# shanice-l/UNOPose

Measured on AMD Instinct MI355X. Metric: (query,ref) pairs/sec forward, higher is better.
Workload: dtype bf16; 1 GPU; UNOPose.forward, batch 32 pairs/GPU, 2048 query pts, 5000->2048 reference pts, 196 coarse pts, 518x518 crops, DINOv2 ViT-B/14 reg4, random-init (trained-like) weights

## Files before the change

### include/unopose_hip.h

```cpp
#ifndef UNOPOSE_HIP_H
#define UNOPOSE_HIP_H

#include <stdint.h>

#ifdef __cplusplus
extern "C" {
#endif

#define UNOPOSE_OK 0
#define UNOPOSE_EINVAL 1
#define UNOPOSE_ELAUNCH 2
#define UNOPOSE_ENOMEM 3

typedef void *unopose_stream_t;

int unopose_abi_version(void);
const char *unopose_last_error(void);


int unopose_furthest_point_sampling(const float *xyz, int B, int N, int M,
                                    int32_t *idx, unopose_stream_t stream);

int unopose_gather_points(const float *points, const int32_t *idx, int B, int C,
                          int N, int M, float *out, unopose_stream_t stream);

int unopose_gather_points_grad(const float *grad_out, const int32_t *idx, int B,
                               int C, int N, int M, float *grad_points,
                               unopose_stream_t stream);

int unopose_ball_query(const float *new_xyz, const float *xyz, int B, int N,
                       int M, float radius, int nsample, int32_t *idx,
                       unopose_stream_t stream);

int unopose_group_points(const float *points, const int32_t *idx, int B, int C,
                         int N, int M, int S, float *out,
                         unopose_stream_t stream);

int unopose_group_points_grad(const float *grad_out, const int32_t *idx, int B,
                              int C, int N, int M, int S, float *grad_points,
                              unopose_stream_t stream);

int unopose_three_nn(const float *unknown, const float *known, int B, int n,
                     int m, float *dist2, int32_t *idx, unopose_stream_t stream);

int unopose_three_interpolate(const float *points, const int32_t *idx,
                              const float *weight, int B, int c, int m, int n,
                              float *out, unopose_stream_t stream);

int unopose_three_interpolate_grad(const float *grad_out, const int32_t *idx,
                                   const float *weight, int B, int c, int n,
                                   int m, float *grad_points,
                                   unopose_stream_t stream);


int unopose_lrf_global(const float *pts, int B, int N, int use_ref_rad,
                       float *out, unopose_stream_t stream);

int unopose_query_lrf_group(const float *xyz, int B, int N, float radius,
                            int nsample, float *out, unopose_stream_t stream);

int unopose_lrf_group_idx(const float *xyz, const float *new_xyz, const int *idx,
                          int B, int N, float radius, int nsample, float *out,
                          unopose_stream_t stream);

int unopose_weighted_procrustes(const float *src, const float *ref,
                                const float *w, int M, int N, float thresh,
                                float eps, float *R, float *t,
                                unopose_stream_t stream);

int unopose_pe_image_bytes(void);
int unopose_pe_pack_weights(const float *w1, const float *b1, const float *w2, const float *b2,
                            const float *w3, const float *b3, void *image, unopose_stream_t stream);
int unopose_pe_group_mlp_max_packed(const float *xyz, int B, int N, float radius, int nsample,
                                    const void *image, float *out, unopose_stream_t stream);

int unopose_pe_group_mlp_max_packed_cand(const float *xyz, int B, int N, float radius, int nsample,
                                         const void *image, const int *cand_in, const int *cand_cnt_in,
                                         int cand_stride, int *cand_out, int *cand_cnt_out, float *out,
                                         unopose_stream_t stream);
int unopose_pe_group_mlp_max_packed_out(const float *xyz, int B, int N, float radius, int nsample, const void *image,
                                        const int *cand_in, const int *cand_cnt_in, int cand_stride, int *cand_out,
                                        int *cand_cnt_out, void *out, int out_ld, int out_split, unopose_stream_t stream);

int unopose_geo_embedding(const float *points, int B, int n, const void *wd_hi,
                          const void *wd_lo, const void *wa_hi, const void *wa_lo,
                          const float *bias_sum, const float *div_term,
                          float sigma_d, float factor_a, int reduce_mean, int split,
                          int out_bf16, int32_t *knn_ws, void *out,
                          unopose_stream_t stream);

int unopose_geo_embedding_table(const float *points, int B, int n, const float *tab_d, int rows_d, const float *tab_a, int rows_a,
                                const float *bias_sum, const float *w_d, const float *div_term, int hinv, int npoint, float sigma_d,
                                float factor_a, int reduce_mean, int out_bf16, int32_t *knn_ws, void *out,
                                unopose_stream_t stream);

int unopose_geo_embedding_train_workgroups(int B, int n);
int unopose_geo_embedding_train_forward(const float *points, int B, int n, const float *tab_d, int rows_d, const float *tab_a, int rows_a,
                                        const float *bias_sum, const float *w_d, const float *div_term, int hinv, float sigma_d, float factor_a,
                                        int reduce_mean, int32_t *knn, float *out, void *amax, unopose_stream_t stream);
int unopose_geo_embedding_train_backward(const float *points, const int32_t *knn, int B, int n, int rows_d, int rows_a, int hinv, float sigma_d,
                                         float factor_a, int reduce_mean, const float *dE, const void *amax, float *ws, float *full_d,
                                         int *past_table, unopose_stream_t stream);

int unopose_pe_group_mlp_max(const float *xyz, int B, int N, float radius, int nsample,
                             const float *w1, const float *b1, const float *w2,
                             const float *b2, const float *w3, const float *b3,
                             int bf16x3, float *out, unopose_stream_t stream);

int unopose_softmax_stats(const float *x, int B, int R, int C, float *stats_ws, unopose_stream_t stream);
int unopose_infonce_grad(const float *x, int B, int R, int C, const float *stats_ws, const long long *label1,
                         const long long *label2, const float *g, float *grad, unopose_stream_t stream);

int unopose_bn_train_chunk(void);
int unopose_bn_relu_train_forward(const float *x, int B, int C, long L, const float *gamma, const float *beta, float eps, float momentum,
                                  float *running_mean, float *running_var, float *workspace, float *mean, float *rstd, float *y,
                                  unopose_stream_t stream);
int unopose_bn_relu_train_backward(const float *x, const float *dy, int B, int C, long L, const float *gamma, const float *beta,
                                   const float *mean, const float *rstd, float *workspace, float *dgamma, float *dbeta, float *dx,
                                   unopose_stream_t stream);

int unopose_bn_relu_maxpool_train_forward(const float *x, int B, int C, int N, int S, const float *gamma, const float *beta, float eps,
                                          float momentum, float *running_mean, float *running_var, float *workspace, float *mean, float *rstd,
                                          float *out, int32_t *idx, unopose_stream_t stream);
int unopose_bn_relu_maxpool_train_backward(const float *x, const float *g, const int32_t *idx, int B, int C, int N, int S, const float *gamma,
                                           const float *beta, const float *mean, const float *rstd, float *workspace, float *dgamma, float *dbeta,
                                           float *dx, unopose_stream_t stream);

int unopose_saliency_train_forward(const float *atten, const float *s1, const float *s2, int B, int n1, int n2, float *m1, float *m2, float *rmax,
                                   float *rsum, float *cmax, float *csum, unopose_stream_t stream);
int unopose_saliency_train_backward(const float *atten, const float *s1, const float *s2, const float *m1, const float *m2, const float *rmax,
                                    const float *rsum, const float *cmax, const float *csum, const float *g1, const float *g2, int B, int n1, int n2,
                                    float *d_atten, float *ds1, float *ds2, unopose_stream_t stream);

int unopose_nearest_partner(const float *a, const float *b, int B, int n, int m, int over_b, float thr, float *dmin, int32_t *arg,
                            uint8_t *any_close, unopose_stream_t stream);

int unopose_conv1x1_train_wgrad_blocks(void);
int unopose_conv1x1_train_forward(const float *x, int B, int cin, long L, const float *w, int cout, float *y, unopose_stream_t stream);
int unopose_conv1x1_train_wgrad(const float *dy, const float *x, int B, int cout, int cin, long L, float *workspace, float *dw,
                                unopose_stream_t stream);

int unopose_linear_wgrad_f32_splits(long rows, int N, int K);
int unopose_linear_wgrad_f32(const float *g, const float *x, long rows, int N, int K, float *workspace, float *dw, unopose_stream_t stream);
int unopose_assign_labels(const float *atten, int B, int R, int C, const float *score1,
                          const float *score2, float *stats_ws, float *w1, float *w2,
                          unopose_stream_t stream);

int unopose_fine_correspondences(const float *atten, int B, int R, int C, const float *score1,
                                 const float *score2, const float *stats_ws, const float *w1,
                                 const float *w2, const float *pts2, float *weight, float *pred,
                                 unopose_stream_t stream);

int unopose_upproj_plan(const long long *choose, int B2, int Np, int H, int W, int side, int tok_offset, int tok_stride,
                        int cap_rows, int *ws, int *row_list, int *cellmap, int *tile_info, unopose_stream_t stream);

int unopose_linear_bf16_ld(const void *A, int lda, const void *W, int ldw, const float *bias, void *C, int ldc, long M, int N, int K,
                           int epilogue, unopose_stream_t stream);

int unopose_linear_add_layernorm_bf16(const void *A, const void *W, const float *bias, const void *resid, const float *ln_w,
                                      const float *ln_b, float eps, void *C, long M, int K, unopose_stream_t stream);

int unopose_linear_bf16_kv_vt(const void *A, const void *W, const float *bias, void *C, void *vt, long M, int N, int K, int tokens, int key_pad,
                              unopose_stream_t stream);

int unopose_linear_bf16_gather(const void *A, long M, int K, const void *W, int N, const float *bias, const int *row_list,
                               const int *tile_info, int max_tiles, void *C, unopose_stream_t stream);

int unopose_bilinear_sample_compact(const void *Cc, const int *cellmap, const long long *choose, int B2, int side, int Np,
                                    int H, int W, void *out, int out_bf16, unopose_stream_t stream);

int unopose_fine_assign(const void *f1, const void *f2, int B, int R, int C, int D, float shift, const float *score1,
                        const float *score2, const float *pts2, float *ws, float *w1, float *w2, float *weight,
                        float *pred, unopose_stream_t stream);

int unopose_min_dist(const float *p, const float *q, int B, int N, int M, const float *R,
                     const float *t, int cand_per_b, float *out, unopose_stream_t stream);

int unopose_coarse_hypotheses(const float *atten, int B, int R, int C, const float *score1,
                              const float *score2, const float *stats_ws, const float *w1,
                              const float *w2, const float *rand, int nprop, const float *pts1,
                              const float *pts2, float *cdf_ws, float *Rout, float *tout,
                              float *dis, unopose_stream_t stream);

int unopose_coarse_scores(const float *pts1, const float *pts2, int B, int n1, int n2,
                          const float *Rall, const float *tall, int nprop, const int64_t *top,
                          int ncand, const float *w1, float *score, unopose_stream_t stream);

int unopose_topk_smallest(const float *x, int B, int n, int k, int64_t *idx, unopose_stream_t stream);
int unopose_coarse_pick(const float *score, const int64_t *top, int B, int ncand, const float *Rall, const float *tall, int nprop,
                        float *R, float *t, float *best_score, unopose_stream_t stream);

int unopose_token_attention(const void *q, int ldq, const void *k, int ldk, const void *vt,
                            const void *qp, int ldqp, const void *E, int B, int n, int m,
                            float scale, void *out, unopose_stream_t stream);
int unopose_token_attention_key_pad(void);

int unopose_token_attention_f32(const float *q, int ldq, const float *k, int ldk, const float *vt,
                                const float *qp, int ldqp, const float *E, int B, int n, int m,
                                float scale, float *out, unopose_stream_t stream);
int unopose_vit_attention_f32(const float *qkv, int B, int T, int H, float *out, unopose_stream_t stream);
int unopose_token_attention_f32_train(const float *q, int ldq, const float *k, int ldk, const float *vt,
                                      const float *qp, int ldqp, const float *E, int B, int n, int m,
                                      float scale, float *out, float *P, unopose_stream_t stream);
int unopose_token_attention_f32_backward(const float *dout, const float *q, int ldq, const float *v, int ldv,
                                         const float *kt, const float *qp, int ldqp, const float *E, const float *P,
                                         int B, int n, int m, float scale, float *dS, float *dq, float *dk, float *dv,
                                         float *dqp, float *dE, unopose_stream_t stream);
int unopose_vit_attention_f32_split(const float *qkv, int B, int T, int H, void *out_split, unopose_stream_t stream);
int unopose_vit_attention_f32_ss(const void *qkv_split, int B, int T, int H, void *out_split, unopose_stream_t stream);

int unopose_vit_attention(const void *qkv, int B, int T, int H, void *out, unopose_stream_t stream);

int unopose_add_layernorm(const void *a, int a_bf16, const void *b, int b_bf16, const float *w,
                          const float *bias, long rows, int C, float eps, void *out, int out_bf16,
                          unopose_stream_t stream);

int unopose_add_layernorm_strided(const void *a, int a_bf16, const void *b, int b_bf16, const float *w,
                                  const float *bias, long rows, int C, float eps, void *out, int out_bf16,
                                  long ld_out, unopose_stream_t stream);

int unopose_bilinear_sample(const void *z, int z_bf16, const long long *choose, int B, int side, int Np,
                            int H, int W, float *out, unopose_stream_t stream);

int unopose_bilinear_sample_tokens(const void *z, int z_bf16, const long long *choose, int B, int side, int Np,
                                   int H, int W, int tok_offset, int tok_stride, float *out,
                                   unopose_stream_t stream);

int unopose_scale_residual_layernorm(float *x, const void *y_bf16, const float *gamma, const float *w,
                                     const float *bias, long rows, int C, float eps, void *out_bf16,
                                     unopose_stream_t stream);
int unopose_scale_residual_layernorm_f32(float *x, const float *y, const float *gamma, const float *w, const float *bias, long rows,
                                         int C, float eps, void *out_split, long out_ld_bytes, unopose_stream_t stream);

int unopose_scale_residual(float *x, const void *y_bf16, const float *gamma, long rows, int C,
                           unopose_stream_t stream);

int unopose_linear_attention(const void *x, const float *inv_softplus_scale, const void *kvt,
                             const float *ksum, int B, int N, int focus, int mode, void *out,
                             unopose_stream_t stream);
int unopose_linear_attention_kv_state(const void *ykv, const float *inv_softplus_scale, int B, int J, int rows_per_pair,
                                      int first_row, int focus, void *kvt, float *ksum, unopose_stream_t stream);
int unopose_linear_attention_f32(const float *x, const float *inv_softplus_scale, const float *kvt,
                                 const float *ksum, int B, int N, int focus, int mode, float *out,
                                 unopose_stream_t stream);

int unopose_render_depth(const float *verts, int V, const int *faces, int F, const float *Rt, const float *K4, int P, int H, int W,
                         float *depth, unopose_stream_t stream);

int unopose_patchify_bf16(const float *rgb_a, int na, const float *rgb_b, int nb, int S, int Kp, void *out,
                          unopose_stream_t stream);
int unopose_vit_tokens_layernorm(const void *patch, const float *pos, const float *prefix, int npre, int P, int nimg, int C,
                                 const float *ln_w, const float *ln_b, float eps, float *x, void *n1, float *row_mean, unopose_stream_t stream);
int unopose_patchify_split(const float *rgb_a, int na, const float *rgb_b, int nb, int S, int Kp, void *out, unopose_stream_t stream);
int unopose_vit_tokens_layernorm_f32(const float *patch, const float *pos, const float *prefix, int npre, int P, int nimg, int C,
                                     const float *ln_w, const float *ln_b, float eps, float *x, void *n1_split, unopose_stream_t stream);
int unopose_row_dot(const void *x, int x_bf16, const float *w, float b, long rows, int C, void *out, int out_bf16,
                    unopose_stream_t stream);
int unopose_normalize_rows_bf16(const void *x, int x_bf16, long rows, int C, float temp, void *out, int out_f32,
                                unopose_stream_t stream);
int unopose_gather_rows(const void *feats, int B, int N, int row_bytes, const void *idx, int idx_is_i64, int J, int off,
                        const void *alt, long alt_stride_bytes, int prepend, void *out, unopose_stream_t stream);
int unopose_transpose_pad_bf16(const void *v, long ld, int B, int m, int C, int pad, void *vt, unopose_stream_t stream);
int unopose_transpose_pad_f32(const float *v, long ld, int B, int m, int C, int pad, float *vt, unopose_stream_t stream);

int unopose_cloud_radius(const float *pts, int B, int N, float *radius, unopose_stream_t stream);
int unopose_scale_by_radius(const float *x, int B, int n, const float *radius, float eps, int multiply, float *out, unopose_stream_t stream);
int unopose_overlap_scores(const void *scores, int x_bf16, int B, int n_tot, int n1, int halves, float *out, unopose_stream_t stream);
int unopose_nan_to_num_multi(const void *ptrs_dev, const void *sizes_dev, int n_tensors, long max_size, float nan_value, float posinf_value,
                             float neginf_value, unopose_stream_t stream);
int unopose_copy_rows(const void *src, long src_stride_bytes, void *dst, long dst_stride_bytes, int rows, int row_bytes,
                      unopose_stream_t stream);
int unopose_rigid_rows_bf16(const float *p, int B, int N, const float *t, const float *R, void *out, unopose_stream_t stream);
int unopose_token_sum_bf16(const void *x, int B, int J, int C, float *out, unopose_stream_t stream);
int unopose_pose_score(const float *dis, const float *w, int B, int N, float thr, float *out, unopose_stream_t stream);

int unopose_linear_bf16(const void *A, const void *W, const float *bias, void *C, long M, int N, int K,
                        int epilogue, unopose_stream_t stream);
int unopose_gemm_bf16_tile(void);

int unopose_linear_bf16_residual(const void *A, const void *W, const float *bias, float *xres, void *xb, float *stats, const float *prev,
                                 int prev_nparts, long M, int N, int K, unopose_stream_t stream);
int unopose_linear_bf16_lnfold(const void *A, const void *W, const float *dvec, const float *cvec, const float *stats, int nparts, float eps,
                               void *C, long M, int N, int K, int gelu, unopose_stream_t stream);
int unopose_gemm_fold_stagger(int eighth_ticks_per_ktile);

int unopose_bmm_f32(const float *A, long sab, long sah, long sai, long sak, const float *Bm, long sbb, long sbh, long sbj, long sbk,
                    float *C, int bo, int bi, int n, int m, int K, float alpha, unopose_stream_t stream);

int unopose_split_bf16x2(const float *X, long M, int K, void *Xs, unopose_stream_t stream);
int unopose_linear_f32x3(const void *As, const void *Ws, const float *bias, float *C, void *Cs, long M, int N, int K,
                         int epilogue, unopose_stream_t stream);
int unopose_linear_f32x3_bf16(const void *As, const void *Ws, const float *bias, const void *resid, void *Cb, long M, int N, int K,
                              unopose_stream_t stream);

#ifdef __cplusplus
}
#endif
#endif
```

### unopose_amd/_lib.py

```python
import ctypes
import os

import torch

_HERE = os.path.dirname(os.path.abspath(__file__))
SO_PATH = os.environ.get("UNOPOSE_LIB") or os.path.join(_HERE, "libunopose_hip.so")

_lib = None

_P = ctypes.c_void_p
_I = ctypes.c_int
_F = ctypes.c_float
_L = ctypes.c_long

SIGNATURES = {
    "unopose_furthest_point_sampling": [_P, _I, _I, _I, _P, _P],
    "unopose_gather_points": [_P, _P, _I, _I, _I, _I, _P, _P],
    "unopose_gather_points_grad": [_P, _P, _I, _I, _I, _I, _P, _P],
    "unopose_ball_query": [_P, _P, _I, _I, _I, _F, _I, _P, _P],
    "unopose_group_points": [_P, _P, _I, _I, _I, _I, _I, _P, _P],
    "unopose_group_points_grad": [_P, _P, _I, _I, _I, _I, _I, _P, _P],
    "unopose_three_nn": [_P, _P, _I, _I, _I, _P, _P, _P],
    "unopose_three_interpolate": [_P, _P, _P, _I, _I, _I, _I, _P, _P],
    "unopose_three_interpolate_grad": [_P, _P, _P, _I, _I, _I, _I, _P, _P],
    "unopose_lrf_global": [_P, _I, _I, _I, _P, _P],
    "unopose_query_lrf_group": [_P, _I, _I, _F, _I, _P, _P],
    "unopose_lrf_group_idx": [_P, _P, _P, _I, _I, _F, _I, _P, _P],
    "unopose_weighted_procrustes": [_P, _P, _P, _I, _I, _F, _F, _P, _P, _P],
    "unopose_assign_labels": [_P, _I, _I, _I, _P, _P, _P, _P, _P, _P],
    "unopose_linear_bf16_ld": [_P, _I, _P, _I, _P, _P, _I, ctypes.c_long, _I, _I, _I, _P],
    "unopose_scale_residual_layernorm_f32": [_P, _P, _P, _P, _P, ctypes.c_long, _I, _F, _P, _L, _P],
    "unopose_gather_rows": [_P, _I, _I, _I, _P, _I, _I, _I, _P, _L, _I, _P, _P],
    "unopose_softmax_stats": [_P, _I, _I, _I, _P, _P],
    "unopose_infonce_grad": [_P, _I, _I, _I, _P, _P, _P, _P, _P, _P],
    "unopose_fine_correspondences": [_P, _I, _I, _I, _P, _P, _P, _P, _P, _P, _P, _P, _P],
    "unopose_upproj_plan": [_P, _I, _I, _I, _I, _I, _I, _I, _I, _P, _P, _P, _P, _P],
    "unopose_linear_add_layernorm_bf16": [_P, _P, _P, _P, _P, _P, _F, _P, ctypes.c_long, _I, _P],
    "unopose_linear_bf16_kv_vt": [_P, _P, _P, _P, _P, ctypes.c_long, _I, _I, _I, _I, _P],
    "unopose_linear_bf16_gather": [_P, ctypes.c_long, _I, _P, _I, _P, _P, _P, _I, _P, _P],
    "unopose_bilinear_sample_compact": [_P, _P, _P, _I, _I, _I, _I, _I, _P, _I, _P],
    "unopose_fine_assign": [_P, _P, _I, _I, _I, _I, _F, _P, _P, _P, _P, _P, _P, _P, _P, _P],
    "unopose_min_dist": [_P, _P, _I, _I, _I, _P, _P, _I, _P, _P],
    "unopose_coarse_hypotheses": [_P, _I, _I, _I, _P, _P, _P, _P, _P, _P, _I, _P, _P, _P, _P, _P, _P, _P],
    "unopose_coarse_scores": [_P, _P, _I, _I, _I, _P, _P, _I, _P, _I, _P, _P, _P],
    "unopose_topk_smallest": [_P, _I, _I, _I, _P, _P],
    "unopose_coarse_pick": [_P, _P, _I, _I, _P, _P, _I, _P, _P, _P, _P],
    "unopose_token_attention": [_P, _I, _P, _I, _P, _P, _I, _P, _I, _I, _I, _F, _P, _P],
    "unopose_token_attention_key_pad": [],
    "unopose_token_attention_f32": [_P, _I, _P, _I, _P, _P, _I, _P, _I, _I, _I, _F, _P, _P],
    "unopose_token_attention_f32_train": [_P, _I, _P, _I, _P, _P, _I, _P, _I, _I, _I, _F, _P, _P, _P],
    "unopose_token_attention_f32_backward": [_P, _P, _I, _P, _I, _P, _P, _I, _P, _P, _I, _I, _I, _F, _P, _P, _P, _P, _P, _P, _P],
    "unopose_vit_attention_f32": [_P, _I, _I, _I, _P, _P],
    "unopose_vit_attention_f32_split": [_P, _I, _I, _I, _P, _P],
    "unopose_vit_attention_f32_ss": [_P, _I, _I, _I, _P, _P],
    "unopose_bn_train_chunk": [],
    "unopose_bn_relu_train_forward": [_P, _I, _I, ctypes.c_long, _P, _P, _F, _F, _P, _P, _P, _P, _P, _P, _P],
    "unopose_bn_relu_train_backward": [_P, _P, _I, _I, ctypes.c_long, _P, _P, _P, _P, _P, _P, _P, _P, _P],
    "unopose_bn_relu_maxpool_train_forward": [_P, _I, _I, _I, _I, _P, _P, _F, _F, _P, _P, _P, _P, _P, _P, _P, _P],
    "unopose_bn_relu_maxpool_train_backward": [_P, _P, _P, _I, _I, _I, _I, _P, _P, _P, _P, _P, _P, _P, _P, _P],
    "unopose_nearest_partner": [_P, _P, _I, _I, _I, _I, _F, _P, _P, _P, _P],
    "unopose_saliency_train_forward": [_P, _P, _P, _I, _I, _I, _P, _P, _P, _P, _P, _P, _P],
    "unopose_saliency_train_backward": [_P, _P, _P, _P, _P, _P, _P, _P, _P, _P, _P, _I, _I, _I, _P, _P, _P, _P],
    "unopose_conv1x1_train_wgrad_blocks": [],
    "unopose_conv1x1_train_forward": [_P, _I, _I, ctypes.c_long, _P, _I, _P, _P],
    "unopose_conv1x1_train_wgrad": [_P, _P, _I, _I, _I, ctypes.c_long, _P, _P, _P],
    "unopose_linear_wgrad_f32_splits": [ctypes.c_long, _I, _I],
    "unopose_linear_wgrad_f32": [_P, _P, ctypes.c_long, _I, _I, _P, _P, _P],
    "unopose_vit_attention": [_P, _I, _I, _I, _P, _P],
    "unopose_add_layernorm": [_P, _I, _P, _I, _P, _P, ctypes.c_long, _I, _F, _P, _I, _P],
    "unopose_add_layernorm_strided": [_P, _I, _P, _I, _P, _P, ctypes.c_long, _I, _F, _P, _I, ctypes.c_long, _P],
    "unopose_bilinear_sample": [_P, _I, _P, _I, _I, _I, _I, _I, _P, _P],
    "unopose_bilinear_sample_tokens": [_P, _I, _P, _I, _I, _I, _I, _I, _I, _I, _P, _P],
    "unopose_scale_residual_layernorm": [_P, _P, _P, _P, _P, ctypes.c_long, _I, _F, _P, _P],
    "unopose_scale_residual": [_P, _P, _P, ctypes.c_long, _I, _P],
    "unopose_linear_attention": [_P, _P, _P, _P, _I, _I, _I, _I, _P, _P],
    "unopose_linear_attention_f32": [_P, _P, _P, _P, _I, _I, _I, _I, _P, _P],
    "unopose_linear_attention_kv_state": [_P, _P, _I, _I, _I, _I, _I, _P, _P, _P],
    "unopose_linear_bf16": [_P, _P, _P, _P, ctypes.c_long, _I, _I, _I, _P],
    "unopose_gemm_bf16_tile": [],
    "unopose_gemm_fold_stagger": [_I],
    "unopose_linear_bf16_residual": [_P, _P, _P, _P, _P, _P, _P, _I, ctypes.c_long, _I, _I, _P],
    "unopose_linear_bf16_lnfold": [_P, _P, _P, _P, _P, _I, _F, _P, ctypes.c_long, _I, _I, _I, _P],
    "unopose_patchify_bf16": [_P, _I, _P, _I, _I, _I, _P, _P],
    "unopose_patchify_split": [_P, _I, _P, _I, _I, _I, _P, _P],
    "unopose_vit_tokens_layernorm": [_P, _P, _P, _I, _I, _I, _I, _P, _P, _F, _P, _P, _P, _P],
    "unopose_vit_tokens_layernorm_f32": [_P, _P, _P, _I, _I, _I, _I, _P, _P, _F, _P, _P, _P],
    "unopose_row_dot": [_P, _I, _P, _F, ctypes.c_long, _I, _P, _I, _P],
    "unopose_normalize_rows_bf16": [_P, _I, ctypes.c_long, _I, _F, _P, _I, _P],
    "unopose_transpose_pad_bf16": [_P, ctypes.c_long, _I, _I, _I, _I, _P, _P],
    "unopose_transpose_pad_f32": [_P, _L, _I, _I, _I, _I, _P, _P],
    "unopose_cloud_radius": [_P, _I, _I, _P, _P],
    "unopose_scale_by_radius": [_P, _I, _I, _P, _F, _I, _P, _P],
    "unopose_overlap_scores": [_P, _I, _I, _I, _I, _I, _P, _P],
    "unopose_copy_rows": [_P, _L, _P, _L, _I, _I, _P],
    "unopose_nan_to_num_multi": [_P, _P, _I, _L, _F, _F, _F, _P],
    "unopose_rigid_rows_bf16": [_P, _I, _I, _P, _P, _P, _P],
    "unopose_token_sum_bf16": [_P, _I, _I, _I, _P, _P],
    "unopose_pose_score": [_P, _P, _I, _I, _F, _P, _P],
    "unopose_render_depth": [_P, _I, _P, _I, _P, _P, _I, _I, _I, _P, _P],
    "unopose_bmm_f32": [_P, ctypes.c_long, ctypes.c_long, ctypes.c_long, ctypes.c_long, _P, ctypes.c_long, ctypes.c_long, ctypes.c_long, ctypes.c_long, _P, _I, _I, _I, _I, _I, _F, _P],
    "unopose_split_bf16x2": [_P, ctypes.c_long, _I, _P, _P],
    "unopose_linear_f32x3": [_P, _P, _P, _P, _P, ctypes.c_long, _I, _I, _I, _P],
    "unopose_pe_image_bytes": [],
    "unopose_pe_pack_weights": [_P, _P, _P, _P, _P, _P, _P, _P],
    "unopose_pe_group_mlp_max_packed": [_P, _I, _I, _F, _I, _P, _P, _P],
    "unopose_pe_group_mlp_max_packed_cand": [_P, _I, _I, _F, _I, _P, _P, _P, _I, _P, _P, _P, _P],
    "unopose_pe_group_mlp_max_packed_out": [_P, _I, _I, _F, _I, _P, _P, _P, _I, _P, _P, _P, _I, _I, _P],
    "unopose_linear_f32x3_bf16": [_P, _P, _P, _P, _P, ctypes.c_long, _I, _I, _P],
    "unopose_pe_group_mlp_max": [_P, _I, _I, _F, _I, _P, _P, _P, _P, _P, _P, _I, _P, _P],
    "unopose_geo_embedding": [_P, _I, _I, _P, _P, _P, _P, _P, _P, _F, _F, _I, _I, _I, _P, _P, _P],
    "unopose_geo_embedding_train_workgroups": [_I, _I],
    "unopose_geo_embedding_train_forward": [_P, _I, _I, _P, _I, _P, _I, _P, _P, _P, _I, _F, _F, _I, _P, _P, _P, _P],
    "unopose_geo_embedding_train_backward": [_P, _P, _I, _I, _I, _I, _I, _F, _F, _I, _P, _P, _P, _P, _P, _P],
    "unopose_geo_embedding_table": [_P, _I, _I, _P, _I, _P, _I, _P, _P, _P, _I, _I, _F, _F, _I, _I, _P, _P, _P],
}


def lib():
    global _lib
    if _lib is None:
        if not os.path.exists(SO_PATH):
            raise RuntimeError(
                f"{SO_PATH} is missing: the HIP extension has not been built "
                "(run `python -m unopose_amd.build`). There is no CPU fallback."
            )
        L = ctypes.CDLL(SO_PATH)
        L.unopose_abi_version.restype = _I
        L.unopose_last_error.restype = ctypes.c_char_p
        for name, argtypes in SIGNATURES.items():
            fn = getattr(L, name)
            fn.argtypes = argtypes
            fn.restype = _I
        _lib = L
    return _lib


def stream_ptr(device=None):
    if device is None:
        idx = torch._C._cuda_getDevice()
    else:
        idx = device if isinstance(device, int) else torch.device(device).index
        if idx is None:
            idx = torch._C._cuda_getDevice()
    return ctypes.c_void_p(torch._C._cuda_getCurrentRawStream(idx))


class _NullContext:
    def __enter__(self):
        return None

    def __exit__(self, *a):
        return False


_NULL_CONTEXT = _NullContext()


def on_device(dev):
    idx = dev.index if isinstance(dev, torch.device) else dev
    if idx is None or idx == torch._C._cuda_getDevice():
        return _NULL_CONTEXT
    return torch.cuda.device(idx)


def call(name, *args):
    L = lib()
    rc = getattr(L, name)(*args)
    if rc != 0:
        raise RuntimeError(f"{name} failed (code {rc}): {L.unopose_last_error().decode()}")


def ptr(t):
    return ctypes.c_void_p(t.data_ptr())


def check_f32(x, name):
    if not x.is_cuda:
        raise RuntimeError(f"{name}: CPU not supported")
    if not x.is_contiguous():
        raise RuntimeError(f"{name} must be a contiguous tensor")
    if x.dtype != torch.float32:
        raise RuntimeError(f"{name} must be a float tensor")


def check_i32(x, name):
    if not x.is_cuda:
        raise RuntimeError(f"{name} must be a CUDA tensor")
    if not x.is_contiguous():
        raise RuntimeError(f"{name} must be a contiguous tensor")
    if x.dtype != torch.int32:
        raise RuntimeError(f"{name} must be an int tensor")
```

### unopose_amd/csrc/pe.hip

```cpp
#include "common.h"
#include "jacobi3.h"

namespace unopose {

constexpr int PE_SCAN_STEPS = 4;

__device__ __forceinline__ int cd_row(int r, int h) { return (r & 3) + 8 * (r >> 2) + 4 * h; }

constexpr int PE_GDIM = 8, PE_GCELLS = PE_GDIM * PE_GDIM * PE_GDIM;
struct PeGrid {
  float ox, oy, oz, ihx, ihy, ihz;
  int nx, ny, nz;
  const u16 *start;
  const u16 *order;
  uint32_t *bits;
};
__device__ __forceinline__ int pe_cell(float v, float o, float ih, int n) { return max(0, min(n - 1, (int)((v - o) * ih))); }

template <typename NT>
__device__ __forceinline__ int pe_centre_frame(const float *sx, const float *sy, const float *sz, int N, int S,
                                               float radius, float r2, int lane, float cx, float cy, float cz,
                                               NT *nbr, Vec3 &xp, Vec3 &yp, Vec3 &zp, const int *cand = nullptr,
                                               int ncand = -1, const PeGrid *grid = nullptr) {
  int cnt = 0, first = 0;
  if (grid && ncand < 0) {
    const int W = (N + 31) >> 5;
    for (int w = lane; w < W; w += 64) grid->bits[w] = 0u;
    const int icx = pe_cell(cx, grid->ox, grid->ihx, grid->nx), icy = pe_cell(cy, grid->oy, grid->ihy, grid->ny),
              icz = pe_cell(cz, grid->oz, grid->ihz, grid->nz);
    int rs = 0, re = 0;
    if (lane < 9) {
      const int y = icy + lane % 3 - 1, z = icz + lane / 3 - 1;
      if (y >= 0 && y < grid->ny && z >= 0 && z < grid->nz) {
        const int row = (z * grid->ny + y) * grid->nx;
        rs = grid->start[row + max(icx - 1, 0)];
        re = grid->start[row + min(icx + 1, grid->nx - 1) + 1];
      }
    }
    __builtin_amdgcn_fence(__ATOMIC_RELEASE, "wavefront");
    __builtin_amdgcn_wave_barrier();
    __builtin_amdgcn_fence(__ATOMIC_ACQUIRE, "wavefront");
#pragma unroll 1
    for (int i = 0; i < 9; ++i) {
      const int s0 = __builtin_amdgcn_readlane(rs, i), e0 = __builtin_amdgcn_readlane(re, i);
      for (int q = s0 + lane; q < e0; q += 64) {
        const int k = grid->order[q];
        const float x = sx[k], y = sy[k], z = sz[k];
        const float d2 = (cx - x) * (cx - x) + (cy - y) * (cy - y) + (cz - z) * (cz - z);
        if (d2 < r2) atomicOr(&grid->bits[k >> 5], 1u << (k & 31));
      }
    }
    __builtin_amdgcn_fence(__ATOMIC_RELEASE, "wavefront");
    __builtin_amdgcn_wave_barrier();
    __builtin_amdgcn_fence(__ATOMIC_ACQUIRE, "wavefront");
    for (int w0 = 0; w0 < W; w0 += 64) {
      const int w = w0 + lane;
      uint32_t bits = w < W ? grid->bits[w] : 0u;
      const int pc = __builtin_popcount(bits);
      int incl = pc;
#pragma unroll
      for (int d = 1; d < 64; d <<= 1) {
        const int t = __shfl_up(incl, d);
        if (lane >= d) incl += t;
      }
      int pos = cnt + incl - pc;
      while (bits) {
        const int bpos = __builtin_ctz(bits);
        bits &= bits - 1u;
        if (pos < S) nbr[pos] = (NT)(32 * w + bpos);
        ++pos;
      }
      cnt += __builtin_amdgcn_readlane(incl, 63);
    }
    __builtin_amdgcn_fence(__ATOMIC_RELEASE, "wavefront");
    __builtin_amdgcn_wave_barrier();
    __builtin_amdgcn_fence(__ATOMIC_ACQUIRE, "wavefront");
    if (cnt > 0) first = nbr[0];
  } else {
  const int nscan = ncand >= 0 ? ncand : N;
  int k0 = 0;
  constexpr int U = PE_SCAN_STEPS;
  for (; k0 < nscan && cnt < S; k0 += 64 * U) {
    int kk[U];
    unsigned long long mask[U];
    bool hit[U];
#pragma unroll
    for (int u = 0; u < U; ++u) {
      int k = k0 + 64 * u + lane;
      hit[u] = false;
      if (k < nscan) {
        if (ncand >= 0) k = cand[k];
        const float x = sx[k], y = sy[k], z = sz[k];
        const float d2 = (cx - x) * (cx - x) + (cy - y) * (cy - y) + (cz - z) * (cz - z);
        hit[u] = d2 < r2;
      }
      kk[u] = k;
      mask[u] = __ballot(hit[u]);
    }
#pragma unroll
    for (int u = 0; u < U; ++u) {
      if (mask[u]) {
        const int pre =
            (int)__builtin_amdgcn_mbcnt_hi((uint32_t)(mask[u] >> 32), __builtin_amdgcn_mbcnt_lo((uint32_t)mask[u], 0u));
        const int pos = cnt + pre;
        if (hit[u] && pos < S) nbr[pos] = (NT)kk[u];
        if (cnt == 0) {
          const int fl = __builtin_ctzll(mask[u]);
          first = ncand >= 0 ? __builtin_amdgcn_readlane(kk[u], fl) : k0 + 64 * u + fl;
        }
        cnt += __builtin_popcountll(mask[u]);
      }
    }
  }
  if (k0 < nscan) cnt = S + 1;
  }
  for (int l = min(cnt, S) + lane; l < S; l += 64) nbr[l] = (NT)first;
  __builtin_amdgcn_fence(__ATOMIC_RELEASE, "wavefront");
  __builtin_amdgcn_wave_barrier();
  __builtin_amdgcn_fence(__ATOMIC_ACQUIRE, "wavefront");

  float a00 = 0, a01 = 0, a02 = 0, a11 = 0, a12 = 0, a22 = 0;
  for (int l = lane; l < S; l += 64) {
    const int k = nbr[l];
    const float x = cx - sx[k], y = cy - sy[k], z = cz - sz[k];
    a00 += x * x; a01 += x * y; a02 += x * z; a11 += y * y; a12 += y * z; a22 += z * z;
  }
  const float inv_s = 1.f / (float)S;
  a00 = wave_sum_f32(a00) * inv_s; a01 = wave_sum_f32(a01) * inv_s; a02 = wave_sum_f32(a02) * inv_s;
  a11 = wave_sum_f32(a11) * inv_s; a12 = wave_sum_f32(a12) * inv_s; a22 = wave_sum_f32(a22) * inv_s;
  Vec3 e0, e1, z0;
  float l0, l1, l2;
  eig_sym3(a00, a01, a02, a11, a12, a22, e0, e1, z0, l0, l1, l2);
  int vote = 0;
  for (int l0i = 0; l0i < S; l0i += 64) {
    const int l = l0i + lane;
    float pr = 0.f;
    if (l < S) {
      const int k = nbr[l];
      pr = z0.x * (cx - sx[k]) + z0.y * (cy - sy[k]) + z0.z * (cz - sz[k]);
    }
    vote += __builtin_popcountll(__ballot(pr > 1e-3f)) - __builtin_popcountll(__ballot(pr < -1e-3f));
  }
  zp = vote < 0 ? scale(z0, -1.f) : z0;
  float vx = 0, vy = 0, vz = 0;
  for (int l = lane; l < S; l += 64) {
    const int k = nbr[l];
    const Vec3 xn = v3(sx[k] - cx, sy[k] - cy, sz[k] - cz);
    const float nrm = dot(zp, xn);
    const Vec3 vi = sub(xn, scale(zp, nrm));
    float alpha = radius - sqrtf(dot(xn, xn));
    alpha *= alpha;
    const float ab = alpha * (nrm * nrm);
    vx += ab * vi.x; vy += ab * vi.y; vz += ab * vi.z;
  }
  vx = wave_sum_f32(vx); vy = wave_sum_f32(vy); vz = wave_sum_f32(vz);
  const float nacc = sqrtf(vx * vx + vy * vy + vz * vz) + 1e-10f;
  xp = v3(vx / nacc, vy / nacc, vz / nacc);
  yp = cross(xp, zp);
  return cnt;
}

struct PeLds {
  float w1[6 * 32];
  float w2[32 * 64];
  float w3[64 * 128];
  float b1[32], b2[64], b3[128];
};

__global__ __launch_bounds__(256) void pe_group_mlp_max_kernel(
    const float *__restrict__ xyz, int N, float radius, int S, int cpw, const float *__restrict__ w1,
    const float *__restrict__ b1, const float *__restrict__ w2, const float *__restrict__ b2,
    const float *__restrict__ w3, const float *__restrict__ b3, float *__restrict__ out) {
  extern __shared__ float4 smem4[];
  PeLds *L = reinterpret_cast<PeLds *>(smem4);
  float *sx = reinterpret_cast<float *>(L + 1);
  float *sy = sx + N, *sz = sy + N;
  int *nbr_all = reinterpret_cast<int *>(sz + N);
  float *stage_all = reinterpret_cast<float *>(nbr_all + 4 * S);
  const int b = blockIdx.y, tid = threadIdx.x, lane = tid & 63, wave = tid >> 6;
  const int half = lane >> 5, col = lane & 31;
  int *nbr = nbr_all + wave * S;
  float *stage = stage_all + wave * 128;
  const float *P = xyz + (size_t)b * N * 3;

  for (int e = tid; e < N * 3; e += 256) {
    const float v = P[e];
    const int p = e / 3, comp = e - p * 3;
    (comp == 0 ? sx : comp == 1 ? sy : sz)[p] = v;
  }
  for (int e = tid; e < 32 * 6; e += 256) L->w1[(e % 6) * 32 + e / 6] = w1[e];
  for (int e = tid; e < 64 * 32; e += 256) L->w2[(e % 32) * 64 + e / 32] = w2[e];
  for (int e = tid; e < 128 * 64; e += 256) L->w3[(e % 64) * 128 + e / 64] = w3[e];
  if (tid < 32) L->b1[tid] = b1[tid];
  if (tid < 64) L->b2[tid] = b2[tid];
  if (tid < 128) L->b3[tid] = b3[tid];
  __syncthreads();
  const float r2 = radius * radius;

  for (int ci = 0; ci < cpw; ++ci) {
    const int j = (blockIdx.x * 4 + wave) * cpw + ci;
    if (j >= N) break;
    const float cx = sx[j], cy = sy[j], cz = sz[j];
    Vec3 xp, yp, zp;
    const int cnt_nb = pe_centre_frame(sx, sy, sz, N, S, radius, r2, lane, cx, cy, cz, nbr, xp, yp, zp);
    const int S_eff = min(S, (max(min(cnt_nb, S), 1) + 31) & ~31);

    f32x16 rmax[4];
#pragma unroll
    for (int t = 0; t < 4; ++t)
#pragma unroll
      for (int r = 0; r < 16; ++r) rmax[t][r] = 0.f;
    for (int t0 = 0; t0 < S_eff; t0 += 32) {
      const int k = nbr[t0 + col];
      const float dx = sx[k] - cx, dy = sy[k] - cy, dz = sz[k] - cz;
      const Vec3 q = v3(dx / radius, dy / radius, dz / radius);
      const float lx = dot(xp, q), ly = dot(yp, q), lz = dot(zp, q);
      f32x16 h1;
#pragma unroll
      for (int r = 0; r < 16; ++r) h1[r] = 0.f;
      h1 = __builtin_amdgcn_mfma_f32_32x32x2f32(L->w1[(0 + half) * 32 + col], half ? dy : dx, h1, 0, 0, 0);
      h1 = __builtin_amdgcn_mfma_f32_32x32x2f32(L->w1[(2 + half) * 32 + col], half ? lx : dz, h1, 0, 0, 0);
      h1 = __builtin_amdgcn_mfma_f32_32x32x2f32(L->w1[(4 + half) * 32 + col], half ? lz : ly, h1, 0, 0, 0);
#pragma unroll
      for (int r = 0; r < 16; ++r) h1[r] = fmaxf(h1[r] + L->b1[cd_row(r, half)], 0.f);
      f32x16 h2[2];
#pragma unroll
      for (int ot = 0; ot < 2; ++ot) {
#pragma unroll
        for (int r = 0; r < 16; ++r) h2[ot][r] = 0.f;
#pragma unroll
        for (int r = 0; r < 16; ++r)
          h2[ot] = __builtin_amdgcn_mfma_f32_32x32x2f32(L->w2[cd_row(r, half) * 64 + ot * 32 + col], h1[r], h2[ot], 0,
                                                       0, 0);
#pragma unroll
        for (int r = 0; r < 16; ++r) h2[ot][r] = fmaxf(h2[ot][r] + L->b2[ot * 32 + cd_row(r, half)], 0.f);
      }
#pragma unroll
      for (int ot = 0; ot < 4; ++ot) {
        f32x16 h3;
#pragma unroll
        for (int r = 0; r < 16; ++r) h3[r] = 0.f;
#pragma unroll
        for (int it = 0; it < 2; ++it)
#pragma unroll
          for (int r = 0; r < 16; ++r)
            h3 = __builtin_amdgcn_mfma_f32_32x32x2f32(L->w3[(it * 32 + cd_row(r, half)) * 128 + ot * 32 + col],
                                                      h2[it][r], h3, 0, 0, 0);
#pragma unroll
        for (int r = 0; r < 16; ++r)
          rmax[ot][r] = fmaxf(rmax[ot][r], fmaxf(h3[r] + L->b3[ot * 32 + cd_row(r, half)], 0.f));
      }
    }
#pragma unroll
    for (int t = 0; t < 4; ++t)
#pragma unroll
      for (int r = 0; r < 16; ++r) {
        float v = rmax[t][r];
        v = fmaxf(v, dpp_f32<0x111, 0xF>(v, 0.f));
        v = fmaxf(v, dpp_f32<0x112, 0xF>(v, 0.f));
        v = fmaxf(v, dpp_f32<0x114, 0xF>(v, 0.f));
        v = fmaxf(v, dpp_f32<0x118, 0xF>(v, 0.f));
        v = fmaxf(v, dpp_f32<0x142, 0xA>(v, 0.f));
        if (col == 31) stage[t * 32 + cd_row(r, half)] = v;
      }
    __builtin_amdgcn_fence(__ATOMIC_RELEASE, "wavefront");
    __builtin_amdgcn_wave_barrier();
    __builtin_amdgcn_fence(__ATOMIC_ACQUIRE, "wavefront");
    float *O = out + ((size_t)b * N + j) * 128;
    O[lane] = stage[lane];
    O[lane + 64] = stage[lane + 64];
    __builtin_amdgcn_wave_barrier();
  }
}

__device__ __forceinline__ int pe_kperm(int c) {
  const int cc = c & 15;
  return (c & ~15) + ((cc >> 2) & 1) * 8 + (cc & 3) + 4 * (cc >> 3);
}

struct PeLdsB {
  u16 w1h[32][24], w1l[32][24];
  u16 w2h[64][40], w2l[64][40];
  u16 w3h[128][64], w3l[128][64];
  float b1[32], b2[64], b3[128];
};

__global__ __launch_bounds__(256) void pe_pack_weights_kernel(const float *__restrict__ w1, const float *__restrict__ b1,
                                                              const float *__restrict__ w2, const float *__restrict__ b2,
                                                              const float *__restrict__ w3, const float *__restrict__ b3,
                                                              PeLdsB *__restrict__ L) {
  const int tid = threadIdx.x;
  for (int e = tid; e < 32 * 16; e += 256) {
    const int o = e >> 4, kk = e & 15;
    const float v = kk < 6 ? w1[o * 6 + kk] : 0.f;
    const u16 h = f2bf(v);
    L->w1h[o][kk] = h;
    L->w1l[o][kk] = f2bf(v - bf2f(h));
  }
  for (int e = tid; e < 64 * 32; e += 256) {
    const int o = e >> 5, c = e & 31;
    const float v = w2[e];
    const u16 h = f2bf(v);
    L->w2h[o][pe_kperm(c)] = h;
    L->w2l[o][pe_kperm(c)] = f2bf(v - bf2f(h));
  }
  for (int e = tid; e < 128 * 64; e += 256) {
    const int o = e >> 6, c = e & 63;
    const float v = w3[e];
    const u16 h = f2bf(v);
    const int kp = pe_kperm(c) ^ ((o & 7) << 3);
    L->w3h[o][kp] = h;
    L->w3l[o][kp] = f2bf(v - bf2f(h));
  }
  if (tid < 32) L->b1[tid] = b1[tid];
  if (tid < 64) L->b2[tid] = b2[tid];
  if (tid < 128) L->b3[tid] = b3[tid];
}

constexpr int PE_NW = 4;
__global__ __launch_bounds__(PE_NW * 64, 8 / PE_NW) void pe_group_mlp_max_bf16x3_kernel(
    const float *__restrict__ xyz, int N, float radius, int S, int cpw, const uint4 *__restrict__ image,
    const int *__restrict__ cand_in, const int *__restrict__ cand_cnt_in, int cand_stride, int *__restrict__ cand_out,
    int *__restrict__ cand_cnt_out, float *__restrict__ out, int out_ld, int out_split, int use_grid) {
  extern __shared__ float4 smem4[];
  PeLdsB *L = reinterpret_cast<PeLdsB *>(smem4);
  float *sx = reinterpret_cast<float *>(L + 1);
  float *sy = sx + N, *sz = sy + N;
  float *stage_all = sz + N;
  u16 *nbr_all = reinterpret_cast<u16 *>(stage_all + PE_NW * 128);
  u16 *gstart = nbr_all + PE_NW * S;
  u16 *gorder = gstart + PE_GCELLS + 2;
  const int b = blockIdx.y, tid = threadIdx.x, lane = tid & 63, wave = tid >> 6;
  const int half = lane >> 5, col = lane & 31;
  u16 *nbr = nbr_all + wave * S;
  float *stage = stage_all + wave * 128;
  const float *P = xyz + (size_t)b * N * 3;

  for (int e = tid; e < N * 3; e += PE_NW * 64) {
    const float v = P[e];
    const int p = e / 3, comp = e - p * 3;
    (comp == 0 ? sx : comp == 1 ? sy : sz)[p] = v;
  }
  for (int e = tid; e < (int)(sizeof(PeLdsB) / 16); e += PE_NW * 64) smem4[e] = *reinterpret_cast<const float4 *>(image + e);
  __syncthreads();
  const float r2 = radius * radius;
  PeGrid grid;
  if (use_grid) {
    static_assert(PE_NW * 128 >= PE_GCELLS, "the cell counters borrow the staging area");
    uint32_t *cnt32 = reinterpret_cast<uint32_t *>(stage_all);
    float *red = reinterpret_cast<float *>(nbr_all);
    float lo[3] = {3e38f, 3e38f, 3e38f}, hi[3] = {-3e38f, -3e38f, -3e38f};
    for (int p = tid; p < N; p += PE_NW * 64) {
      lo[0] = fminf(lo[0], sx[p]), hi[0] = fmaxf(hi[0], sx[p]);
      lo[1] = fminf(lo[1], sy[p]), hi[1] = fmaxf(hi[1], sy[p]);
      lo[2] = fminf(lo[2], sz[p]), hi[2] = fmaxf(hi[2], sz[p]);
    }
#pragma unroll
    for (int a = 0; a < 3; ++a) {
      lo[a] = -wave_max_f32(-lo[a]);
      hi[a] = wave_max_f32(hi[a]);
      if (lane == 0) red[wave * 6 + a] = lo[a], red[wave * 6 + 3 + a] = hi[a];
    }
    for (int c = tid; c < PE_GCELLS; c += PE_NW * 64) cnt32[c] = 0u;
    __syncthreads();
    float org[3], ih[3];
    int nd[3];
#pragma unroll
    for (int a = 0; a < 3; ++a) {
      float l = red[a], h = red[3 + a];
      for (int w = 1; w < PE_NW; ++w) l = fminf(l, red[w * 6 + a]), h = fmaxf(h, red[w * 6 + 3 + a]);
      const float ext = h - l, h0 = radius * 1.001f;
      int n = (int)(ext / h0) + 1;
      float edge = h0;
      if (!(n <= PE_GDIM)) n = PE_GDIM, edge = fmaxf(h0, ext / (float)PE_GDIM * 1.001f);
      org[a] = __int_as_float(__builtin_amdgcn_readfirstlane(__float_as_int(l)));
      ih[a] = __int_as_float(__builtin_amdgcn_readfirstlane(__float_as_int(1.f / edge)));
      nd[a] = __builtin_amdgcn_readfirstlane(max(n, 1));
    }
    grid.ox = org[0], grid.oy = org[1], grid.oz = org[2], grid.ihx = ih[0], grid.ihy = ih[1], grid.ihz = ih[2];
    grid.nx = nd[0], grid.ny = nd[1], grid.nz = nd[2];
    grid.start = gstart, grid.order = gorder, grid.bits = reinterpret_cast<uint32_t *>(stage);
    auto cell_of = [&](int p) {
      return (pe_cell(sz[p], grid.oz, grid.ihz, grid.nz) * grid.ny + pe_cell(sy[p], grid.oy, grid.ihy, grid.ny)) * grid.nx +
             pe_cell(sx[p], grid.ox, grid.ihx, grid.nx);
    };
    for (int p = tid; p < N; p += PE_NW * 64) atomicAdd(&cnt32[cell_of(p)], 1u);
    __syncthreads();
    {
      constexpr int CPT = PE_GCELLS / (PE_NW * 64);
      static_assert(CPT * PE_NW * 64 == PE_GCELLS, "cells divide among the threads");
      uint32_t c[CPT], sum = 0;
#pragma unroll
      for (int e = 0; e < CPT; ++e) c[e] = cnt32[tid * CPT + e], sum += c[e];
      uint32_t incl = sum;
#pragma unroll
      for (int d = 1; d < 64; d <<= 1) {
        const uint32_t t = __shfl_up(incl, d);
        if (lane >= d) incl += t;
      }
      uint32_t *wtot = reinterpret_cast<uint32_t *>(red) + 32;
      if (lane == 63) wtot[wave] = incl;
      __syncthreads();
      uint32_t base = incl - sum;
      for (int w = 0; w < wave; ++w) base += wtot[w];
#pragma unroll
      for (int e = 0; e < CPT; ++e) {
        gstart[tid * CPT + e] = (u16)base;
        cnt32[tid * CPT + e] = base;
        base += c[e];
      }
      if (tid == PE_NW * 64 - 1) gstart[PE_GCELLS] = (u16)base;
    }
    __syncthreads();
    for (int p = tid; p < N; p += PE_NW * 64) gorder[atomicAdd(&cnt32[cell_of(p)], 1u)] = (u16)p;
    __syncthreads();
  }

  for (int ci = 0; ci < cpw; ++ci) {
    const int j = (blockIdx.x * PE_NW + wave) * cpw + ci;
    if (j >= N) break;
    const float cx = sx[j], cy = sy[j], cz = sz[j];
    Vec3 xp, yp, zp;
    const int *cand = nullptr;
    int ncand = -1;
    if (cand_in) {
      ncand = cand_cnt_in[(size_t)b * N + j];
      cand = cand_in + ((size_t)b * N + j) * cand_stride;
    }
    const int cnt = pe_centre_frame(sx, sy, sz, N, S, radius, r2, lane, cx, cy, cz, nbr, xp, yp, zp, cand, ncand, use_grid ? &grid : nullptr);
    if (cand_out) {
      int *co = cand_out + ((size_t)b * N + j) * S;
      for (int l = lane; l < S; l += 64) co[l] = nbr[l];
      if (lane == 0) cand_cnt_out[(size_t)b * N + j] = cnt <= S ? cnt : -1;
    }

    f32x16 rmax[4];
#pragma unroll
    for (int t = 0; t < 4; ++t)
#pragma unroll
      for (int r = 0; r < 16; ++r) rmax[t][r] = 0.f;
    const int S_eff = min(S, (max(min(cnt, S), 1) + 31) & ~31);
    for (int t0 = 0; t0 < S_eff; t0 += 32) {
      asm volatile("" ::: "memory");
      const int k = nbr[t0 + col];
      const float dx = sx[k] - cx, dy = sy[k] - cy, dz = sz[k] - cz;
      const Vec3 q = v3(dx / radius, dy / radius, dz / radius);
      float f[8] = {dx, dy, dz, dot(xp, q), dot(yp, q), dot(zp, q), 0.f, 0.f};
      if (half) {
#pragma unroll
        for (int e = 0; e < 8; ++e) f[e] = 0.f;
      }
      const bf16x8_hl x = split8_bf16(f);
      struct Grp {
        bf16x8_hl w[4];
        float4 b[4];
      } ga, gb;
      auto load_l1 = [&](Grp &g) {
        g.w[0].hi = *reinterpret_cast<const bf16x8 *>(&L->w1h[col][half * 8]);
        g.w[0].lo = *reinterpret_cast<const bf16x8 *>(&L->w1l[col][half * 8]);
#pragma unroll
        for (int q = 0; q < 4; ++q) g.b[q] = *reinterpret_cast<const float4 *>(&L->b1[8 * q + 4 * half]);
      };
      auto load_l2 = [&](Grp &g, int ot) {
#pragma unroll
        for (int ks = 0; ks < 2; ++ks) {
          g.w[ks].hi = *reinterpret_cast<const bf16x8 *>(&L->w2h[ot * 32 + col][ks * 16 + half * 8]);
          g.w[ks].lo = *reinterpret_cast<const bf16x8 *>(&L->w2l[ot * 32 + col][ks * 16 + half * 8]);
        }
#pragma unroll
        for (int q = 0; q < 4; ++q) g.b[q] = *reinterpret_cast<const float4 *>(&L->b2[ot * 32 + 8 * q + 4 * half]);
      };
      auto load_l3 = [&](Grp &g, int ot) {
        const int row = ot * 32 + col;
#pragma unroll
        for (int ks = 0; ks < 4; ++ks) {
          const int kp = (ks * 16 + half * 8) ^ ((row & 7) << 3);
          g.w[ks].hi = *reinterpret_cast<const bf16x8 *>(&L->w3h[row][kp]);
          g.w[ks].lo = *reinterpret_cast<const bf16x8 *>(&L->w3l[row][kp]);
        }
#pragma unroll
        for (int q = 0; q < 4; ++q) g.b[q] = *reinterpret_cast<const float4 *>(&L->b3[ot * 32 + 8 * q + 4 * half]);
      };
      auto init = [&](f32x16 &h, const Grp &g) {
#pragma unroll
        for (int q = 0; q < 4; ++q) {
          h[4 * q + 0] = g.b[q].x;
          h[4 * q + 1] = g.b[q].y;
          h[4 * q + 2] = g.b[q].z;
          h[4 * q + 3] = g.b[q].w;
        }
      };
      bf16x8_hl a1[2], a2[4];
      auto relu_split = [&](const f32x16 &h, bf16x8_hl *o) {
#pragma unroll
        for (int s2 = 0; s2 < 2; ++s2) {
          float v[8];
#pragma unroll
          for (int e = 0; e < 8; ++e) v[e] = fmaxf(h[s2 * 8 + e], 0.f);
          o[s2] = split8_bf16(v);
        }
      };
      load_l1(ga);
      load_l2(gb, 0);
      __builtin_amdgcn_sched_barrier(0);
      {
        f32x16 h1;
        init(h1, ga);
        h1 = mfma3_hh_hl_lh_32x32(ga.w[0], x, h1);
        load_l2(ga, 1);
        __builtin_amdgcn_sched_barrier(0);
        relu_split(h1, a1);
      }
      {
        f32x16 h2;
        init(h2, gb);
#pragma unroll
        for (int ks = 0; ks < 2; ++ks) h2 = mfma3_hh_hl_lh_32x32(gb.w[ks], a1[ks], h2);
        load_l3(gb, 0);
        __builtin_amdgcn_sched_barrier(0);
        relu_split(h2, a2);
        init(h2, ga);
#pragma unroll
        for (int ks = 0; ks < 2; ++ks) h2 = mfma3_hh_hl_lh_32x32(ga.w[ks], a1[ks], h2);
        load_l3(ga, 1);
        __builtin_amdgcn_sched_barrier(0);
        relu_split(h2, a2 + 2);
      }
#pragma unroll
      for (int ot = 0; ot < 4; ++ot) {
        Grp &g = (ot & 1) ? ga : gb;
        f32x16 h3;
        init(h3, g);
#pragma unroll
        for (int ks = 0; ks < 4; ++ks) h3 = mfma3_hh_hl_lh_32x32(g.w[ks], a2[ks], h3);
        if (ot + 2 < 4) {
          load_l3(g, ot + 2);
          __builtin_amdgcn_sched_barrier(0);
        }
#pragma unroll
        for (int r = 0; r < 16; ++r) rmax[ot][r] = fmaxf(rmax[ot][r], h3[r]);
      }
    }
#pragma unroll
    for (int t = 0; t < 4; ++t)
#pragma unroll
      for (int r = 0; r < 16; ++r) {
        float v = rmax[t][r];
        v = fmaxf(v, dpp_f32<0x111, 0xF>(v, 0.f));
        v = fmaxf(v, dpp_f32<0x112, 0xF>(v, 0.f));
        v = fmaxf(v, dpp_f32<0x114, 0xF>(v, 0.f));
        v = fmaxf(v, dpp_f32<0x118, 0xF>(v, 0.f));
        v = fmaxf(v, dpp_f32<0x142, 0xA>(v, 0.f));
        if (col == 31) stage[t * 32 + cd_row(r, half)] = v;
      }
    __builtin_amdgcn_fence(__ATOMIC_RELEASE, "wavefront");
    __builtin_amdgcn_wave_barrier();
    __builtin_amdgcn_fence(__ATOMIC_ACQUIRE, "wavefront");
    float *O = out + ((size_t)b * N + j) * out_ld;
    if (!out_split) {
      O[lane] = stage[lane];
      O[lane + 64] = stage[lane + 64];
    } else {
      uint32_t *O32 = reinterpret_cast<uint32_t *>(O);
#pragma unroll
      for (int q = 0; q < 2; ++q) {
        const int d = lane + 64 * q, blk = d >> 5, w = d & 31, k = blk * 32 + (w & 15) * 2;
        const float v0 = stage[k], v1 = stage[k + 1];
        const uint32_t h = cvt_pk_bf16_f32(v0, v1);
        O32[d] = (w & 16) ? cvt_pk_bf16_lo(v0, v1, h) : h;
      }
    }
    __builtin_amdgcn_wave_barrier();
  }
}

}

using namespace unopose;

extern "C" {

int unopose_pe_image_bytes(void) { return (int)sizeof(PeLdsB); }

int unopose_pe_pack_weights(const float *w1, const float *b1, const float *w2, const float *b2, const float *w3,
                            const float *b3, void *image, unopose_stream_t stream) {
  UNOPOSE_REQUIRE(w1 && b1 && w2 && b2 && w3 && b3 && image, "pe_pack_weights: null pointer");
  hipLaunchKernelGGL(pe_pack_weights_kernel, dim3(1), dim3(256), 0, (hipStream_t)stream, w1, b1, w2, b2, w3, b3,
                     (PeLdsB *)image);
  return check_launch("pe_pack_weights");
}

int unopose_pe_group_mlp_max_packed(const float *xyz, int B, int N, float radius, int nsample, const void *image,
                                    float *out, unopose_stream_t stream) {
  return unopose_pe_group_mlp_max_packed_cand(xyz, B, N, radius, nsample, image, nullptr, nullptr, 0, nullptr, nullptr,
                                              out, stream);
}

int unopose_pe_group_mlp_max_packed_cand(const float *xyz, int B, int N, float radius, int nsample, const void *image,
                                         const int *cand_in, const int *cand_cnt_in, int cand_stride, int *cand_out,
                                         int *cand_cnt_out, float *out, unopose_stream_t stream) {
  return unopose_pe_group_mlp_max_packed_out(xyz, B, N, radius, nsample, image, cand_in, cand_cnt_in, cand_stride, cand_out,
                                             cand_cnt_out, out, 128, 0, stream);
}

int unopose_pe_group_mlp_max_packed_out(const float *xyz, int B, int N, float radius, int nsample, const void *image,
                                        const int *cand_in, const int *cand_cnt_in, int cand_stride, int *cand_out,
                                        int *cand_cnt_out, void *out, int out_ld, int out_split, unopose_stream_t stream) {
  UNOPOSE_REQUIRE(xyz && image && out, "pe_group_mlp_max_packed: null pointer");
  UNOPOSE_REQUIRE(out_ld >= 128 && (out_split == 0 || out_split == 1), "pe_group_mlp_max_packed: bad output stride / mode");
  UNOPOSE_REQUIRE((cand_in == nullptr) == (cand_cnt_in == nullptr) && (cand_out == nullptr) == (cand_cnt_out == nullptr) &&
                      (!cand_in || cand_stride >= 1),
                  "pe_group_mlp_max_packed: candidate list and its counts go together");
  UNOPOSE_REQUIRE(B >= 0 && N >= 1 && nsample >= 32 && nsample % 32 == 0 && B <= 65535,
                  "pe_group_mlp_max_packed: nsample must be a positive multiple of 32 (got %d)", nsample);
  if (B == 0) return UNOPOSE_OK;
  size_t lds = sizeof(PeLdsB) + ((size_t)3 * N + PE_NW * 128) * 4 + (size_t)PE_NW * nsample * 2;
  UNOPOSE_REQUIRE(N < 65536 && lds <= 160 * 1024, "pe_group_mlp_max_packed: N=%d nsample=%d exceed the LDS tile", N, nsample);
  const size_t grid_bytes = ((size_t)PE_GCELLS + 2 + (size_t)N) * 2;
  const int use_grid = radius > 0.f && N <= 4096 && N >= 256 && lds + grid_bytes <= 160 * 1024 && (lds + grid_bytes <= 80 * 1024 || lds > 80 * 1024);
  if (use_grid) lds += grid_bytes;
  lds = (lds + 15) & ~(size_t)15;
  static bool opt[64];
  if (lds_optin(opt, (const void *)pe_group_mlp_max_bf16x3_kernel, 160 * 1024, "pe_group_mlp_max_packed") != UNOPOSE_OK) return UNOPOSE_ELAUNCH;
  const long centres = (long)B * N;
  const int cpw = centres >= 65536 ? 16 : centres >= 32768 ? 8 : centres >= 8192 ? 4 : centres >= 2048 ? 2 : 1;
  dim3 grid(cdiv(N, PE_NW * cpw), B);
  hipLaunchKernelGGL(pe_group_mlp_max_bf16x3_kernel, grid, dim3(PE_NW * 64), lds, (hipStream_t)stream, xyz, N, radius, nsample,
                     cpw, (const uint4 *)image, cand_in, cand_cnt_in, cand_stride, cand_out, cand_cnt_out, (float *)out, out_ld, out_split, use_grid);
  return check_launch("pe_group_mlp_max_packed");
}

int unopose_pe_group_mlp_max(const float *xyz, int B, int N, float radius, int nsample, const float *w1,
                             const float *b1, const float *w2, const float *b2, const float *w3, const float *b3,
                             int bf16x3, float *out, unopose_stream_t stream) {
  UNOPOSE_REQUIRE(xyz && w1 && b1 && w2 && b2 && w3 && b3 && out, "pe_group_mlp_max: null pointer");
  UNOPOSE_REQUIRE(B >= 0 && N >= 1 && nsample >= 32 && nsample % 32 == 0 && B <= 65535,
                  "pe_group_mlp_max: nsample must be a positive multiple of 32 (got %d)", nsample);
  if (B == 0) return UNOPOSE_OK;
  const size_t lds = sizeof(PeLds) + ((size_t)3 * N + 4 * (size_t)nsample + 4 * 128) * 4;
  UNOPOSE_REQUIRE(lds <= 160 * 1024, "pe_group_mlp_max: N=%d nsample=%d exceed the LDS tile", N, nsample);
  static bool opt[64];
  if (lds_optin(opt, (const void *)pe_group_mlp_max_kernel, 160 * 1024, "pe_group_mlp_max") != UNOPOSE_OK) return UNOPOSE_ELAUNCH;
  const long centres = (long)B * N;
  const int cpw = centres >= 32768 ? 8 : centres >= 8192 ? 4 : centres >= 2048 ? 2 : 1;
  dim3 grid(cdiv(N, 4 * cpw), B);
  UNOPOSE_REQUIRE(!bf16x3, "pe_group_mlp_max: the bf16x3 form takes a packed weight image "
                           "(unopose_pe_pack_weights + unopose_pe_group_mlp_max_packed)");
  hipLaunchKernelGGL(pe_group_mlp_max_kernel, grid, dim3(256), lds, (hipStream_t)stream, xyz, N, radius, nsample, cpw,
                     w1, b1, w2, b2, w3, b3, out);
  return check_launch("pe_group_mlp_max");
}

}
```

### unopose_amd/model/modules.py

```python
import math

import torch
import torch.nn as nn
import torch.nn.functional as F

from .. import ops


class _Attention(nn.Module):
    def __init__(self, dim, heads):
        super().__init__()
        self.heads = heads
        self.qkv = nn.Linear(dim, 3 * dim)
        self.proj = nn.Linear(dim, dim)

    def forward(self, x):
        B, T, C = x.shape
        qkv = ops.linear(x, self.qkv)
        o = ops.vit_attention(qkv, self.heads)
        return ops.linear(o, self.proj)


class _LayerScale(nn.Module):
    def __init__(self, dim):
        super().__init__()
        self.gamma = nn.Parameter(torch.full((dim,), 1e-5))


class _Mlp(nn.Module):
    def __init__(self, dim, ratio=4):
        super().__init__()
        self.fc1 = nn.Linear(dim, ratio * dim)
        self.fc2 = nn.Linear(ratio * dim, dim)

    def forward(self, x):
        return ops.mlp(x, self.fc1, self.fc2)


class _Block(nn.Module):
    def __init__(self, dim, heads):
        super().__init__()
        self.norm1 = nn.LayerNorm(dim, eps=1e-6)
        self.attn = _Attention(dim, heads)
        self.ls1 = _LayerScale(dim)
        self.norm2 = nn.LayerNorm(dim, eps=1e-6)
        self.mlp = _Mlp(dim)
        self.ls2 = _LayerScale(dim)

    def forward_fused(self, x, n1, next_norm):
        y = self.attn(n1)
        n2 = ops.scale_residual_layernorm_(x, y, self.ls1.gamma, self.norm2)
        y = self.mlp(n2)
        if next_norm is None:
            ops.scale_residual_(x, y, self.ls2.gamma)
            return x, None
        return x, ops.scale_residual_layernorm_(x, y, self.ls2.gamma, next_norm)

    def forward_folded(self, x, n1, xb, stats):
        a = self.attn
        qkv = ops.linear(n1, a.qkv) if n1 is not None else ops.linear_lnfold(xb, stats, a.qkv, self.norm1)
        xb, stats = ops.linear_residual_(x, ops.vit_attention(qkv, a.heads), a.proj, self.ls1.gamma, stats)
        h = ops.linear_lnfold(xb, stats, self.mlp.fc1, self.norm2, gelu=True)
        return ops.linear_residual_(x, h, self.mlp.fc2, self.ls2.gamma, stats)

    def forward_fused_f32(self, x, n1s, next_norm):
        B, T, C = x.shape
        rows = B * T
        a, m = self.attn, self.mlp
        cq = ops._f32x3_weights(a.qkv)
        qkv_s = ops.linear_f32x3(n1s, cq[1], cq[2], rows, 3 * C, C, out="split")
        cp = ops._f32x3_weights(a.proj)
        y = ops.linear_f32x3(ops.vit_attention_f32_ss(qkv_s, B, T, a.heads), cp[1], cp[2], rows, C, C).reshape(B, T, C)
        n2s = ops.scale_residual_layernorm_f32_(x, y, self.ls1.gamma, self.norm2)
        c1, c2 = ops._f32x3_weights(m.fc1), ops._f32x3_weights(m.fc2)
        hs = ops.linear_f32x3(n2s, c1[1], c1[2], rows, 4 * C, C, gelu=True, out="split")
        y = ops.linear_f32x3(hs, c2[1], c2[2], rows, C, 4 * C).reshape(B, T, C)
        if next_norm is None:
            return ops.scale_residual_layernorm_f32_(x, y, self.ls2.gamma, None), None
        return x, ops.scale_residual_layernorm_f32_(x, y, self.ls2.gamma, next_norm)

    def forward(self, x):
        if torch.is_autocast_enabled() and x.dtype == torch.float32 and x.is_cuda and not ops.is_differentiable():
            x = x.contiguous()
            y = self.attn(ops.add_layernorm(x, None, self.norm1, torch.bfloat16))
            ops.scale_residual_(x, y, self.ls1.gamma)
            y = self.mlp(ops.add_layernorm(x, None, self.norm2, torch.bfloat16))
            return ops.scale_residual_(x, y, self.ls2.gamma)
        x = x + self.attn(self.norm1(x)) * self.ls1.gamma
        return x + self.mlp(self.norm2(x)) * self.ls2.gamma


class _PatchEmbed(nn.Module):
    def __init__(self, dim, patch):
        super().__init__()
        self.proj = nn.Conv2d(3, dim, patch, patch)


SPARSE_SINGLE_CROP = True
F32_PROLOGUE = True
F32_TAPS_SPLIT = True


class SplitTaps:

    def __init__(self, split, B, T, K):
        self.split, self.B, self.T, self.K = split, B, T, K


class ViT(nn.Module):

    def __init__(self, embed_dim=768, depth=12, num_heads=12, patch_size=14, img_size=224, reg_tokens=4):
        super().__init__()
        self.patch_size, self.depth = patch_size, depth
        self.patch_embed = _PatchEmbed(embed_dim, patch_size)
        self.cls_token = nn.Parameter(torch.zeros(1, 1, embed_dim))
        self.reg_token = nn.Parameter(torch.zeros(1, reg_tokens, embed_dim))
        self.pos_embed = nn.Parameter(torch.zeros(1, (img_size // patch_size) ** 2, embed_dim))
        self.blocks = nn.ModuleList([_Block(embed_dim, num_heads) for _ in range(depth)])
        self.norm = nn.LayerNorm(embed_dim, eps=1e-6)
        self.head = nn.Linear(embed_dim, 1000)

    def forward(self, x, taps_side_by_side=False):
        xa, xb = x if isinstance(x, (tuple, list)) else (x, None)
        if ops.vit_prologue_ok(xa, self) and (xb is None or xb.shape[1:] == xa.shape[1:]):
            x, n1, mean = ops.vit_prologue(xa, xb, self, self.blocks[0].norm1, row_mean=True)
            return self._fused_blocks(x, n1, taps_side_by_side, mean)
        if F32_PROLOGUE and ops.vit_prologue_f32_ok(xa, self) and (xb is None or xb.shape[1:] == xa.shape[1:]):
            x, ns = ops.vit_prologue_f32(xa, xb, self, self.blocks[0].norm1)
            return self._fused_blocks_f32(x, ns, taps_side_by_side)
        x = xa if xb is None else torch.cat([xa, xb], 0)
        B = x.shape[0]
        p = self.patch_size
        gh, gw = x.shape[2] // p, x.shape[3] // p
        patches = x.reshape(B, 3, gh, p, gw, p).permute(0, 2, 4, 1, 3, 5).reshape(B, gh * gw, 3 * p * p)
        x = ops.patch_embed(patches, self.patch_embed.proj)
        x = x + self.pos_embed
        x = torch.cat([self.cls_token.expand(B, -1, -1).to(x.dtype), self.reg_token.expand(B, -1, -1).to(x.dtype), x], 1)
        n = self.depth // 4
        taps = {self.depth - 1, self.depth - n - 1, self.depth - 2 * n - 1, self.depth - 3 * n - 1}
        outs = []
        if x.is_cuda and torch.is_autocast_enabled() and x.dtype == torch.float32 and x.shape[-1] % 4 == 0 \
                and not ops.is_differentiable():
            x = x.contiguous()
            return self._fused_blocks(x, ops.add_layernorm(x, None, self.blocks[0].norm1, torch.bfloat16), taps_side_by_side)
        if ops.vit_f32_fused_ok(x, self):
            x = x.contiguous()
            return self._fused_blocks_f32(x, ops.scale_residual_layernorm_f32_(x, None, None, self.blocks[0].norm1), taps_side_by_side)
        for i, blk in enumerate(self.blocks):
            x = blk(x)
            if i in taps:
                outs.append(ops.add_layernorm(x, None, self.norm)
                            if x.is_cuda and torch.is_autocast_enabled() and not ops.is_differentiable() else self.norm(x))
        return outs

    def _fused_blocks_f32(self, x, ns, taps_side_by_side):
        n = self.depth // 4
        taps = {self.depth - 1, self.depth - n - 1, self.depth - 2 * n - 1, self.depth - 3 * n - 1}
        outs = []
        wide = torch.empty(x.shape[0] * x.shape[1], 2 * 4 * x.shape[2], dtype=torch.bfloat16, device=x.device) if taps_side_by_side and F32_TAPS_SPLIT else None
        for i, blk in enumerate(self.blocks):
            x, ns = blk.forward_fused_f32(x, ns, self.blocks[i + 1].norm1 if i + 1 < len(self.blocks) else None)
            if i in taps:
                if wide is not None:
                    ops.scale_residual_layernorm_f32_(x, None, None, self.norm, wide=wide, block=len(outs))
                    outs.append(None)
                else:
                    outs.append(self.norm(x))
        return SplitTaps(wide, x.shape[0], x.shape[1], 4 * x.shape[2]) if wide is not None else outs


def _vit_fused_blocks(self, x, n1, taps_side_by_side, row_mean=None):
    n = self.depth // 4
    taps = {self.depth - 1, self.depth - n - 1, self.depth - 2 * n - 1, self.depth - 3 * n - 1}
    outs = []
    B, _, D = x.shape
    wide = torch.empty(B, x.shape[1], len(taps) * D, dtype=torch.bfloat16, device=x.device) if taps_side_by_side else None
    fold = ops.ln_fold_ok(B * x.shape[1], D, x.device)
    if fold and row_mean is None:
        row_mean = ops.fold_row_means(x)
    xb, stats = None, row_mean
    for i, blk in enumerate(self.blocks):
        nxt = self.blocks[i + 1].norm1 if i + 1 < len(self.blocks) else None
        if fold:
            xb, stats = blk.forward_folded(x, n1, xb, stats)
            n1 = None
        else:
            x, n1 = blk.forward_fused(x, n1, nxt)
        if i in taps:
            k = len(outs)
            outs.append(ops.add_layernorm(x, None, self.norm, out=None if wide is None else wide[:, :, k * D:(k + 1) * D]))
    return outs if wide is None else wide


ViT._fused_blocks = _vit_fused_blocks


def interpolate_pos_embed(pos_embed_ckpt, new_side):
    P0, C = pos_embed_ckpt.shape[-2:]
    s0 = int(P0 ** 0.5)
    if s0 == new_side:
        return pos_embed_ckpt
    t = pos_embed_ckpt.reshape(-1, s0, s0, C).permute(0, 3, 1, 2)
    t = F.interpolate(t, size=(new_side, new_side), mode="bicubic", align_corners=False)
    return t.permute(0, 2, 3, 1).flatten(1, 2)


class ViT_AE(nn.Module):

    def __init__(self, cfg):
        super().__init__()
        assert cfg.up_type == "linear" and cfg.use_pyramid_feat, "only the configured variant is built"
        assert "reg4" in cfg.vit_type and "patch14" in cfg.vit_type
        dims = {"vit_small": (384, 12, 6), "vit_base": (768, 12, 12), "vit_large": (1024, 24, 16)}
        D, depth, heads = dims[cfg.vit_type[:cfg.vit_type.index("_patch")]]
        assert D == cfg.embed_dim
        self.out_dim = cfg.out_dim
        self.img_size = cfg.get("img_size", 224)
        self.vit = ViT(D, depth, heads, 14, self.img_size)
        self.output_upscaling = nn.Linear(4 * D, 16 * cfg.out_dim, bias=True)
        if cfg.get("pretrained", False):
            self.load_dinov2(cfg.vit_ckpt)

    def load_dinov2(self, path):
        ck = torch.load(path, map_location="cpu")["model"]
        sd = self.vit.state_dict()
        for k in ("head.weight", "head.bias"):
            if k in ck and ck[k].shape != sd[k].shape:
                del ck[k]
        if "pos_embed" in ck:
            ck["pos_embed"] = interpolate_pos_embed(ck["pos_embed"], self.img_size // 14)
        self.vit.load_state_dict(ck, strict=False)

    def lowres_map(self, x):
        B, _, H, W = x.shape
        side = H // 14
        outs = self.vit(x)
        z = torch.cat([o[:, 5:, :] for o in outs], dim=2)
        z = ops.linear(z, self.output_upscaling).reshape(B, side, side, 4, 4, self.out_dim)
        return z.permute(0, 1, 3, 2, 4, 5).reshape(B, 4 * side, 4 * side, self.out_dim), (H, W)

    def upprojected(self, x):
        B, _, H, W = x.shape
        side = H // 14
        outs = self.vit(x)
        z = torch.cat([o[:, 5:, :] for o in outs], dim=2)
        return ops.linear(z, self.output_upscaling).reshape(B, side, side, 4, 4, self.out_dim), (H, W)

    def upprojected_tokens(self, x):
        B, _, H, W = x.shape
        return self.upproject(self.vit(x, taps_side_by_side=True), H, W)

    def upproject(self, outs, H, W):
        if isinstance(outs, SplitTaps):
            lin = self.output_upscaling
            c = ops._f32x3_weights(lin)
            z = ops.linear_f32x3(outs.split, c[1], c[2], outs.B * outs.T, lin.weight.shape[0], outs.K)
            return z.reshape(outs.B, outs.T, 4, 4, self.out_dim), (H, W), outs.T - (H // 14) * (W // 14)
        B = outs.shape[0] if torch.is_tensor(outs) else outs[0].shape[0]
        if torch.is_tensor(outs):
            z = ops.linear(outs, self.output_upscaling)
            return z.reshape(B, outs.shape[1], 4, 4, self.out_dim), (H, W), outs.shape[1] - (H // 14) * (W // 14)
        z = ops.linear(torch.cat([o[:, 5:, :] for o in outs], dim=2), self.output_upscaling)
        return z.reshape(B, -1, 4, 4, self.out_dim), (H, W), 0

    def pixel_features(self, x, choose):
        if x.is_cuda and self.out_dim == 256 and not ops.is_differentiable():
            if SPARSE_SINGLE_CROP and ops.sparse_upproj_ok(x) and x.shape[-1] == x.shape[-2] and x.shape[-1] % 14 == 0:
                sd = x.shape[-1] // 14
                npre = self.vit.cls_token.shape[1] + self.vit.reg_token.shape[1]
                plan = ops.upproj_plan(choose, x.shape[-2], x.shape[-1], sd, npre, npre + sd * sd)
                acts = self.vit(x, taps_side_by_side=True)
                if torch.is_tensor(acts) and acts.shape[1] == plan["tok_stride"]:
                    return ops.sparse_pixel_features(acts, self.output_upscaling, plan)
                z, (H, W), off = self.upproject(acts, x.shape[-2], x.shape[-1])
                return ops.bilinear_sample_native(z, choose, H, W, tok_offset=off)
            z, (H, W), off = self.upprojected_tokens(x)
            return ops.bilinear_sample_native(z, choose, H, W, tok_offset=off)
        low, (H, W) = self.lowres_map(x)
        return ops.bilinear_sample_pixels(low, choose, H, W)


class ViTEncoderOneRef(nn.Module):
    def __init__(self, cfg, npoint=None):
        super().__init__()
        self.npoint = npoint
        self.rgb_net = ViT_AE(cfg)


class SinusoidalPositionalEmbedding(nn.Module):
    def __init__(self, d_model):
        super().__init__()
        self.d_model = d_model
        div = torch.exp(torch.arange(0, d_model, 2).float() * (-math.log(10000.0) / d_model))
        self.register_buffer("div_term", div)


class GeometricStructureEmbedding(nn.Module):

    def __init__(self, cfg):
        super().__init__()
        self.sigma_d, self.sigma_a, self.angle_k = cfg.sigma_d, cfg.sigma_a, cfg.angle_k
        self.factor_a = 180.0 / (self.sigma_a * math.pi)
        self.embedding = SinusoidalPositionalEmbedding(cfg.hidden_dim)
        self.proj_d = nn.Linear(cfg.hidden_dim, cfg.hidden_dim)
        self.proj_a = nn.Linear(cfg.hidden_dim, cfg.hidden_dim)
        self.reduction_a = cfg.reduction_a
        if self.reduction_a not in ("max", "mean"):
            raise ValueError(f"Unsupported reduction mode: {self.reduction_a}.")

    def forward(self, points):
        return ops.geo_embedding(points, self)


class _MHA(nn.Module):
    def __init__(self, d, rpe):
        super().__init__()
        self.proj_q = nn.Linear(d, d)
        self.proj_k = nn.Linear(d, d)
        self.proj_v = nn.Linear(d, d)
        if rpe:
            self.proj_p = nn.Linear(d, d)


class _AttentionLayer(nn.Module):
    def __init__(self, d, rpe):
        super().__init__()
        self.attention = _MHA(d, rpe)
        self.linear = nn.Linear(d, d)
        self.norm = nn.LayerNorm(d)


class _AttentionOutput(nn.Module):
    def __init__(self, d):
        super().__init__()
        self.expand = nn.Linear(d, 2 * d)
        self.squeeze = nn.Linear(2 * d, d)
        self.norm = nn.LayerNorm(d)

    def forward(self, x, out=None):
        if x.is_cuda and not ops.is_differentiable():
            return ops.ffn_add_layernorm(x, self.expand, self.squeeze, self.norm, out=out)
        assert out is None
        return self.norm(x + ops.linear(ops.linear(x, self.expand, relu=True), self.squeeze))


class TransformerLayer(nn.Module):

    def __init__(self, d, rpe, heads=4):
        super().__init__()
        self.heads = heads
        self.attention = _AttentionLayer(d, rpe)
        self.output = _AttentionOutput(d)

    def forward(self, x, mem, embed=None, out=None):
        a = self.attention
        if mem is None:
            mem = x
        h = ops.token_attention(x, mem, a.attention, self.heads, embed)
        if x.is_cuda and not ops.is_differentiable():
            x = ops.linear_add_layernorm(h, a.linear, x, a.norm)
        else:
            x = a.norm(ops.linear(h, a.linear) + x)
        return self.output(x, out=out)


class GeometricTransformer(nn.Module):

    def __init__(self, d, heads=4):
        super().__init__()
        self.layers = nn.ModuleList([TransformerLayer(d, True, heads), TransformerLayer(d, False, heads)])

    def forward(self, f0, e0, f1, e1):
        e_all = _adjacent(e0, e1)
        if e_all is not None and f0.shape == f1.shape:
            f = _adjacent(f0, f1)
            f = self.forward_stacked(torch.cat([f0, f1], 0) if f is None else f, e_all)
            B = f0.shape[0]
            return f[:B], f[B:]
        f0 = self.layers[0](f0, f0, e0)
        f1 = self.layers[0](f1, f1, e1)
        f0 = self.layers[1](f0, f1)
        f1 = self.layers[1](f1, f0)
        return f0, f1

    def forward_stacked(self, f, e_all):
        B = f.shape[0] // 2
        f = self.layers[0](f, None, e_all)
        if ops.USE_STACKED_OUT and f.is_cuda and not ops.is_differentiable():
            out = torch.empty_like(f, memory_format=torch.contiguous_format)
            f0 = self.layers[1](f[:B], f[B:], out=out[:B])
            self.layers[1](f[B:], f0, out=out[B:])
            return out
        f0 = self.layers[1](f[:B], f[B:])
        return torch.cat([f0, self.layers[1](f[B:], f0)], 0)


def _adjacent(e0, e1):
    if (e0.shape != e1.shape or e0.dtype != e1.dtype or not e0.is_contiguous() or not e1.is_contiguous()
            or e0.untyped_storage().data_ptr() != e1.untyped_storage().data_ptr()
            or e1.storage_offset() != e0.storage_offset() + e0.numel()):
        return None
    return e0.as_strided((2 * e0.shape[0],) + tuple(e0.shape[1:]), e0.stride())


class _LinearAttention(nn.Module):
    def __init__(self, d):
        super().__init__()
        self.proj_q = nn.Linear(d, d)
        self.proj_k = nn.Linear(d, d)
        self.proj_v = nn.Linear(d, d)
        self.scale = nn.Parameter(torch.zeros(1, 1, d))


class _LinearAttentionLayer(nn.Module):
    def __init__(self, d):
        super().__init__()
        self.attention = _LinearAttention(d)
        self.linear = nn.Linear(d, d)
        self.norm = nn.LayerNorm(d)


class LinearTransformerLayer(nn.Module):

    def __init__(self, d, heads=4, focusing_factor=3):
        super().__init__()
        self.heads, self.focusing_factor = heads, focusing_factor
        self.attention = _LinearAttentionLayer(d)
        self.output = _AttentionOutput(d)

    def forward(self, x, mem, kv_skip=0):
        a = self.attention
        h = ops.focused_linear_attention(x, mem, a.attention, self.heads, self.focusing_factor, kv_skip=kv_skip)
        if x.is_cuda and not ops.is_differentiable():
            x = ops.linear_add_layernorm(h, a.linear, x, a.norm)
        else:
            x = a.norm(ops.linear(h, a.linear) + x)
        return self.output(x)


class SparseToDenseTransformer(nn.Module):

    def __init__(self, d, heads=4, focusing_factor=3):
        super().__init__()
        self.sparse_layer = GeometricTransformer(d, heads)
        self.dense_layer = LinearTransformerLayer(d, heads, focusing_factor)

    @staticmethod
    def _sample(dense, fps_idx):
        return torch.cat([dense[:, 0:1], ops.gather_rows(dense, fps_idx)], dim=1)

    def forward(self, d0, e0, i0, d1, e1, i1):
        f0, f1 = self.sparse_layer(self._sample(d0, i0), e0, self._sample(d1, i1), e1)
        if d0.shape == d1.shape and f0.shape == f1.shape:
            B = d0.shape[0]
            nn_ = self.dense_layer(torch.cat([d0[:, 1:], d1[:, 1:]], 0), torch.cat([f0[:, 1:], f1[:, 1:]], 0))
            n0, n1 = nn_[:B], nn_[B:]
        else:
            n0 = self.dense_layer(d0[:, 1:], f0[:, 1:])
            n1 = self.dense_layer(d1[:, 1:], f1[:, 1:])
        return torch.cat([f0[:, 0:1], n0], 1), torch.cat([f1[:, 0:1], n1], 1)

    def forward_stacked(self, dense, bg, e_all, idx_all):
        f = self.sparse_layer.forward_stacked(ops.gather_rows(dense, idx_all, off=1, alt=bg, prepend=True), e_all)
        if not ops.USE_STACKED_OUT:
            return self.dense_layer(dense, f[:, 1:].contiguous()), f[:, 0:1].contiguous()
        return self.dense_layer(dense, f, kv_skip=1), f[:, 0:1]


class _BN(nn.Module):
    def __init__(self, c):
        super().__init__()
        self.bn = nn.BatchNorm2d(c)


class _ConvBN(nn.Module):
    def __init__(self, cin, cout):
        super().__init__()
        self.conv = nn.Conv2d(cin, cout, 1, bias=False)
        self.normlayer = _BN(cout)

    def folded(self):
        bn = self.normlayer.bn
        s = bn.weight / torch.sqrt(bn.running_var + bn.eps)
        return self.conv.weight.reshape(self.conv.weight.shape[0], -1) * s[:, None], bn.bias - bn.running_mean * s


class _SharedMLP(nn.Module):
    def __init__(self, chans):
        super().__init__()
        for i in range(len(chans) - 1):
            self.add_module(f"layer{i}", _ConvBN(chans[i], chans[i + 1]))
        self.n = len(chans) - 1

    def layers(self):
        return [getattr(self, f"layer{i}") for i in range(self.n)]

    def forward(self, x):
        for l in self.layers():
            x = ops.bn_relu(ops.conv1x1(x, l.conv), l.normlayer.bn)
        return x

    def forward_pooled(self, x):
        ls = self.layers()
        for l in ls[:-1]:
            x = ops.bn_relu(ops.conv1x1(x, l.conv), l.normlayer.bn)
        return ops.bn_relu_maxpool(ops.conv1x1(x, ls[-1].conv), ls[-1].normlayer.bn)


class _Conv1d(nn.Module):
    def __init__(self, cin, cout):
        super().__init__()
        self.conv = nn.Conv1d(cin, cout, 1, bias=True)


class PositionalEncoding(nn.Module):

    def __init__(self, out_dim, r1, r2, nsample1, nsample2):
        super().__init__()
        self.r1, self.r2, self.ns1, self.ns2 = r1, r2, nsample1, nsample2
        self.mlp1 = _SharedMLP([6, 32, 64, 128])
        self.mlp2 = _SharedMLP([6, 32, 64, 128])
        self.mlp3 = _Conv1d(256, out_dim)

    def groups(self, pts):
        pts = pts.float()
        if ops.is_differentiable():
            with torch.autocast("cuda", enabled=False):
                f1 = self.mlp1.forward_pooled(ops.query_lrf_group(pts, self.r1, self.ns1))
                f2 = self.mlp2.forward_pooled(ops.query_lrf_group(pts, self.r2, self.ns2))
            return torch.cat([f1, f2], dim=1).transpose(1, 2)
        if pts.is_cuda and (torch.is_autocast_enabled() or ops.USE_F32X3) and self.r2 >= self.r1 and self.ns1 % 32 == 0 and self.ns2 % 32 == 0:
            f2, cand = ops.pe_group_mlp_max(pts, self.r2, self.ns2, self.mlp2, want_cand=True)
            f1 = ops.pe_group_mlp_max(pts, self.r1, self.ns1, self.mlp1, cand_in=cand)
        else:
            f1 = ops.pe_group_mlp_max(pts, self.r1, self.ns1, self.mlp1)
            f2 = ops.pe_group_mlp_max(pts, self.r2, self.ns2, self.mlp2)
        return torch.cat([f1, f2], dim=2).float()

    def split_ok(self, pts):
        return (pts.is_cuda and torch.is_autocast_enabled() and not ops.is_differentiable() and ops.USE_F32X3 and self.r2 >= self.r1
                and self.ns1 % 32 == 0 and self.ns2 % 32 == 0 and self.mlp3.conv.weight.shape[0] % 256 == 0)

    def groups_split(self, pts, buf, b0):
        pts = pts.float()
        _, cand = ops.pe_group_mlp_max(pts, self.r2, self.ns2, self.mlp2, want_cand=True, out_split=(buf, b0, 128))
        ops.pe_group_mlp_max(pts, self.r1, self.ns1, self.mlp1, cand_in=cand, out_split=(buf, b0, 0))
        return buf

    def _mlp3_split(self):
        conv = self.mlp3.conv
        key = (conv.weight._version, conv.weight.data_ptr(), conv.bias._version)
        cache = getattr(conv, "_f32x3_cache", None)
        if cache is None or cache[0] != key:
            with torch.no_grad():
                cache = (key, ops.split_f32(conv.weight.detach().float().reshape(conv.weight.shape[0], -1).contiguous()),
                         conv.bias.detach().float().contiguous())
            conv._f32x3_cache = cache
        return cache

    def project_add(self, buf, d):
        cache = self._mlp3_split()
        rows = buf.shape[0] * buf.shape[1]
        N, K = self.mlp3.conv.weight.shape[0], buf.shape[2] // 2
        return ops.linear_f32x3_bf16(buf, cache[1], cache[2], rows, N, K, resid=d.contiguous()).reshape(buf.shape[0], buf.shape[1], N)

    def project(self, feat):
        w = self.mlp3.conv.weight.reshape(self.mlp3.conv.weight.shape[0], -1)
        N, K = w.shape
        rows = feat.numel() // K
        with torch.autocast("cuda", enabled=False):
            if feat.is_cuda and not ops.is_differentiable() and ops.f32x3_ok(rows, N, K):
                cache = self._mlp3_split()
                return ops.linear_f32x3(ops.split_f32(feat.float().reshape(rows, K).contiguous()), cache[1], cache[2], rows, N, K).reshape(*feat.shape[:-1], N)
            return F.linear(feat, w.float(), self.mlp3.conv.bias.float())

    def forward(self, pts):
        return self.project(self.groups(pts))
```

### unopose_amd/ops/__init__.py

```python
import sys
import types

from . import _state
from .common import (
    _c, differentiable, is_differentiable, _fallbacks_seen, note_fallback, _params_key, _SPLIT_MEMO, _MUTATION_EPOCH, note_mutation,
    clear_split_memo, _aligned16, _no_autograd, _f32_path, _own_f32, _own_glue,
)
from .dense import (
    linear_backend, _bf16_weights, linear_bf16_hip, own_gemm_ok, bf16_linear_2d, f32x3_ok, split_f32, _f32x3_weights, linear_f32x3,
    linear_f32x3_bf16, linear_f32_raw, _transposed_weights, _LinearFn, _ZERO_BIAS, _zero_bias, linear_train, _lin, mlp, linear,
    ffn_add_layernorm, linear_add_layernorm, patch_embed, vit_prologue_ok, vit_prologue, vit_prologue_f32_ok, vit_prologue_f32, bmm_nt_f32, score_head, add_layernorm,
    scale_residual_, scale_residual_layernorm_f32_, vit_f32_fused_ok, scale_residual_layernorm_, ln_fold_ok, _fold_producer_weights,
    _fold_consumer_weights, linear_residual_, linear_lnfold, fold_shift, fold_row_means, _into,
)
from .attention import (
    vit_attention, vit_attention_f32_split, vit_attention_f32_ss, vit_attention_torch, _KEY_PAD, token_attention,
    _token_attention_hip_f32, _attn_weights, _token_attention_hip, token_attention_torch, _key_pad, _transpose_pad_f32, _TokenAttnFn,
    token_attention_train_ok, _token_attention_train, focused_linear_attention,
    _focused_linear_attention_hip_f32, _focused_linear_attention_hip, focused_linear_attention_torch,
)
from .geometry import (
    lrf_global, query_lrf_group, lrf_group_idx, weighted_procrustes, cloud_radius, scale_by_radius, gather_rows, pairwise_distance,
    _bf16_split, _mfma_fragment_order, _GEO_HINV, _GEO_D_RANGE, _GEO_TABLE_UNAVAILABLE, _geo_tables, geo_embedding, geo_embedding_torch,
    pe_group_mlp_max, pe_group_mlp_max_unfused, furthest_point_sample, _geo_grid, _GeoEmbedFn, geo_embedding_train_ok,
)
from .sampling import (
    bilinear_sample_native, sparse_upproj_ok, upproj_plan, sparse_pixel_features, bilinear_sample_pixels,
)
from .pose import (
    overlap_scores, set_first_rows_, pose_score, rigid_rows, feature_similarity, soft_assignment, coarse_pose_torch, fine_pose_torch, _assign_labels,
    coarse_pose, fine_pose, fine_pose_fused_ok, normalize_rows_bf16, normalize_rows_f32, fine_pose_from_features,
)
from .train import (
    _InfoNCEFn, infonce_two_way, _BNReLUTrain, bn_relu, _BNReLUMaxPoolTrain, bn_relu_maxpool, _SaliencyFn, saliency_pair,
    nearest_partner, _CONV_FWD_PAIRS, _CONV_WGRAD_PAIRS, _conv1x1_pair_ok, _conv1x1_wgrad_ok, _Conv1x1Fn, conv1x1,
)

_SWITCHES = frozenset(['FORBID_LIBRARY_BF16_GEMM', 'GEO_TABLE', 'GEO_TABLE_F32', 'HIP_GEMM_ALL', 'PIXEL_FEATS_BF16', 'TRAIN_FUSED_SALIENCY', 'TRAIN_OWN_ATTN', 'TRAIN_OWN_CONV', 'TRAIN_OWN_GEMM', 'TRAIN_OWN_GEMM_MIN_FLOP', 'TRAIN_OWN_GEO', 'TRAIN_OWN_WGRAD', 'TRAIN_OWN_WGRAD_MIN_ROWS', 'USE_F32X3', 'USE_FUSED_BN_RELU', 'USE_FUSED_FINE', 'USE_FUSED_INFONCE', 'USE_FUSED_LINEAR_LN', 'USE_HIP_GEMM', 'USE_KV_VT', 'USE_LA_KV_STATE', 'USE_LN_FOLD', 'USE_OWN_TOPK', 'USE_SPARSE_UPPROJ', 'USE_STACKED_OUT', '_DIFF'])


class _OpsModule(types.ModuleType):

    def __getattr__(self, name):
        if name in _SWITCHES:
            return getattr(_state, name)
        raise AttributeError(f"module {self.__name__!r} has no attribute {name!r}")

    def __setattr__(self, name, value):
        if name in _SWITCHES:
            setattr(_state, name, value)
        else:
            super().__setattr__(name, value)

    def __delattr__(self, name):
        if name in _SWITCHES:
            raise AttributeError(f"{name} is a switch of ops._state and cannot be deleted")
        super().__delattr__(name)


sys.modules[__name__].__class__ = _OpsModule
```

### unopose_amd/ops/geometry.py

```python
import ctypes

import torch
import torch.nn.functional as F

from .._lib import call, check_f32, lib, on_device, ptr, stream_ptr
from ..pointnet2 import _ext
from . import _state as st
from .common import _c, _own_glue, _params_key, note_fallback
from .dense import _lin, mlp


def lrf_global(pts, use_ref_rad=False):
    pts = _c(pts.float())
    check_f32(pts, "pts")
    B, N, _ = pts.shape
    out = torch.empty_like(pts)
    with on_device(pts.device):
        call("unopose_lrf_global", ptr(pts), B, N, int(bool(use_ref_rad)), ptr(out), stream_ptr())
    return out


def query_lrf_group(xyz, radius, nsample):
    xyz = _c(xyz.float())
    check_f32(xyz, "xyz")
    B, N, _ = xyz.shape
    out = torch.empty(B, 6, N, int(nsample), dtype=torch.float32, device=xyz.device)
    with on_device(xyz.device):
        call("unopose_query_lrf_group", ptr(xyz), B, N, float(radius), int(nsample), ptr(out), stream_ptr())
    return out


def lrf_group_idx(xyz, new_xyz, idx, radius):
    xyz, new_xyz = _c(xyz.float()), _c(new_xyz.float())
    check_f32(xyz, "xyz")
    check_f32(new_xyz, "new_xyz")
    if new_xyz.shape != xyz.shape:
        raise ValueError(f"QueryAndLRFGroup: LRF_batch(xyz, grouped) needs npoint == N, got xyz {tuple(xyz.shape)} "
                         f"new_xyz {tuple(new_xyz.shape)} (pointnet2_utils.py:432-436)")
    idx = _c(idx.to(torch.int32))
    B, N, _ = xyz.shape
    if idx.shape[:2] != (B, N) or not idx.is_cuda:
        raise ValueError(f"idx must be a (B,N,S) device tensor, got {tuple(idx.shape)}")
    S = idx.shape[2]
    out = torch.empty(B, 6, N, S, dtype=torch.float32, device=xyz.device)
    with on_device(xyz.device):
        call("unopose_lrf_group_idx", ptr(xyz), ptr(new_xyz), ptr(idx), B, N, float(radius), S, ptr(out), stream_ptr())
    return out


def weighted_procrustes(src, ref, weights=None, weight_thresh=0.0, eps=1e-5):
    src, ref = _c(src.float()), _c(ref.float())
    check_f32(src, "src_points")
    check_f32(ref, "ref_points")
    M, N, _ = src.shape
    if weights is not None:
        weights = _c(weights.float())
        check_f32(weights, "weights")
    R = torch.empty(M, 3, 3, dtype=torch.float32, device=src.device)
    t = torch.empty(M, 3, dtype=torch.float32, device=src.device)
    with on_device(src.device):
        call("unopose_weighted_procrustes", ptr(src), ptr(ref), ptr(weights) if weights is not None else None, M, N,
             float(weight_thresh), float(eps), ptr(R), ptr(t), stream_ptr())
    return R, t


def cloud_radius(pts):
    if not _own_glue(pts):
        return torch.norm(pts - pts.mean(1, keepdim=True), dim=2).max(1)[0]
    p = _c(pts.float())
    out = torch.empty(p.shape[0], dtype=torch.float32, device=p.device)
    with on_device(p.device):
        call("unopose_cloud_radius", ptr(p), p.shape[0], p.shape[1], ptr(out), stream_ptr())
    return out


def scale_by_radius(x, radius, multiply=False, eps=1e-6):
    if not (_own_glue(x) and x.dtype == torch.float32):
        s = (radius + eps).reshape(-1, *([1] * (x.dim() - 1)))
        return x * s if multiply else x / s
    xc = _c(x)
    out = torch.empty_like(xc)
    B = xc.shape[0]
    if xc.numel() == 0:
        return out
    r = radius.float().reshape(-1)
    if r.numel() != B:
        if r.numel() != 1:
            raise ValueError(f"scale_by_radius: {r.numel()} radii for a batch of {B}")
        r = r.expand(B)
    with on_device(x.device):
        call("unopose_scale_by_radius", ptr(xc), B, xc.numel() // B, ptr(_c(r)), float(eps), int(multiply), ptr(out), stream_ptr())
    return out


def gather_rows(feats, idx, off=0, alt=None, prepend=False, out=None):
    B, N, C = feats.shape
    J = idx.shape[1]
    if (feats.is_cuda and not st._DIFF and not feats.requires_grad and feats.is_contiguous() and idx.is_contiguous() and idx.dtype in (torch.int32, torch.int64)
            and (C * feats.element_size()) % 4 == 0 and B <= 65535):
        alt_stride = 0
        if alt is not None:
            alt = alt.reshape(B, C)
            if alt.dtype != feats.dtype or alt.stride(1) != 1 or 0 < alt.stride(0) < C:
                alt = _c(alt.to(feats.dtype))
            alt_stride = (alt.stride(0) if B > 1 else C) * feats.element_size()
            if alt_stride % 4:
                alt, alt_stride = alt.contiguous(), C * feats.element_size()
        if out is None:
            out = torch.empty(B, J + int(prepend), C, dtype=feats.dtype, device=feats.device)
        else:
            assert out.shape == (B, J + int(prepend), C) and out.dtype == feats.dtype and out.is_contiguous() and out.device == feats.device
        with on_device(feats.device):
            call("unopose_gather_rows", ptr(feats), B, N, C * feats.element_size(), ptr(idx), int(idx.dtype == torch.int64), J, int(off),
                 None if alt is None else ptr(alt), alt_stride, int(prepend), ptr(out), stream_ptr())
        return out
    if out is not None:
        out.copy_(gather_rows(feats, idx, off, alt, prepend))
        return out
    if off == 0 and alt is None:
        return torch.gather(feats, 1, idx.long().unsqueeze(2).expand(-1, -1, C))
    i = idx.long() - off
    g = torch.gather(feats, 1, i.clamp(min=0).unsqueeze(2).expand(-1, -1, C))
    if alt is not None:
        a = alt.reshape(B, 1, C).to(g.dtype)
        g = torch.where((i < 0).unsqueeze(-1), a, g)
        if prepend:
            g = torch.cat([a, g], 1)
    return g


def pairwise_distance(x, y):
    xy = x @ y.transpose(-1, -2)
    return ((x ** 2).sum(-1).unsqueeze(-1) - 2 * xy + (y ** 2).sum(-1).unsqueeze(-2)).clamp(min=0.0)


def _bf16_split(w):
    hi = w.float().to(torch.bfloat16)
    lo = (w.float() - hi.float()).to(torch.bfloat16)
    return hi.contiguous(), lo.contiguous()


def _mfma_fragment_order(w):
    return w.reshape(8, 32, 16, 2, 8).permute(2, 0, 3, 1, 4).contiguous()


_GEO_HINV = 4


_GEO_D_RANGE = 64


_GEO_TABLE_UNAVAILABLE = {}


def _geo_tables(m, key, npoint=4):
    cache = m.__dict__.setdefault("_hip_tables", {})
    c = cache.get(npoint)
    if c is not None and c[0] == key:
        return c[1]
    import math
    lo = npoint // 2 - 1
    rows_a = int(math.floor(math.pi * float(m.factor_a) * _GEO_HINV)) + npoint + 1
    rows_d = _GEO_D_RANGE * _GEO_HINV + npoint
    tabs = None
    if rows_a <= 80 - npoint:
        div = m.embedding.div_term.detach().double()

        def table(rows, lin):
            x = (torch.arange(rows, device=div.device, dtype=torch.float64) - float(lo)) / _GEO_HINV
            om = x[:, None] * div[None, :]
            s = torch.stack([torch.sin(om), torch.cos(om)], dim=-1).reshape(rows, -1)
            return (s @ lin.weight.detach().double().t()).float().contiguous()

        tabs = (table(rows_d, m.proj_d), table(rows_a, m.proj_a), m.proj_d.weight.detach().float().contiguous())
    cache[npoint] = (key, tabs)
    return tabs


def geo_embedding(points, m, out_dtype=None):
    if st._DIFF and torch.is_grad_enabled() and geo_embedding_train_ok(points, m):
        return _GeoEmbedFn.apply(_c(points.detach().float()), m.proj_d.weight, m.proj_d.bias, m.proj_a.weight, m.proj_a.bias, m)
    if st._DIFF or m.proj_d.weight.shape != (256, 256) or m.angle_k != 3 or points.shape[1] < 4:
        if not st._DIFF:
            note_fallback("geo_embedding", f"hidden_dim {tuple(m.proj_d.weight.shape)} / angle_k {m.angle_k} / {points.shape[1]} points (kernel: 256, 3, >= 4)")
        return geo_embedding_torch(points, m)
    points = _c(points.float())
    check_f32(points, "points")
    B, n, _ = points.shape
    if out_dtype is None:
        out_dtype = torch.bfloat16 if torch.is_autocast_enabled() else torch.float32
    bf16_out = out_dtype == torch.bfloat16
    cache = getattr(m, "_hip_cache", None)
    key = (m.proj_d.weight._version, m.proj_a.weight._version, m.proj_d.bias._version, m.proj_a.bias._version, m.proj_d.weight.data_ptr(),
           m.proj_d.weight.device, float(m.factor_a), float(m.sigma_d))
    if cache is None or cache[0] != key:
        assert m.proj_d.weight.shape == (256, 256) and m.angle_k == 3, "kernel is built for hidden_dim=256, k=3"
        wdh, wdl = (_mfma_fragment_order(t) for t in _bf16_split(m.proj_d.weight.detach()))
        wah, wal = (_mfma_fragment_order(t) for t in _bf16_split(m.proj_a.weight.detach()))
        bias = (m.proj_d.bias.detach().float() + m.proj_a.bias.detach().float()).contiguous()
        cache = (key, wdh, wdl, wah, wal, bias, m.embedding.div_term.detach().float().contiguous())
        m._hip_cache = cache
    _, wdh, wdl, wah, wal, bias, div = cache
    out = torch.empty(B, n, n, 256, dtype=out_dtype, device=points.device)
    knn = torch.empty(B, n, 3, dtype=torch.int32, device=points.device)
    if st.GEO_TABLE if bf16_out else st.GEO_TABLE_F32:
        npoint = 4 if bf16_out else 6
        tab = _geo_tables(m, key, npoint)
        if tab is not None and not _GEO_TABLE_UNAVAILABLE.get(points.device, False):
            try:
                with on_device(points.device):
                    call("unopose_geo_embedding_table", ptr(points), B, n, ptr(tab[0]), tab[0].shape[0], ptr(tab[1]), tab[1].shape[0],
                         ptr(bias), ptr(tab[2]), ptr(div), _GEO_HINV, npoint, float(m.sigma_d), float(m.factor_a),
                         int(m.reduction_a == "mean"), int(bf16_out), ptr(knn), ptr(out), stream_ptr())
                return out
            except RuntimeError as e:
                if "cannot reserve" not in str(e):
                    raise
                _GEO_TABLE_UNAVAILABLE[points.device] = True
                note_fallback("geo_embedding", f"table kernel unavailable on {points.device} ({e}): matrix-core kernel")
    with on_device(points.device):
        call("unopose_geo_embedding", ptr(points), B, n, ptr(wdh), ptr(wdl), ptr(wah), ptr(wal), ptr(bias), ptr(div),
             float(m.sigma_d), float(m.factor_a), int(m.reduction_a == "mean"), int(not bf16_out), int(bf16_out),
             ptr(knn), ptr(out), stream_ptr())
    return out


def geo_embedding_torch(points, m):
    points = points.float()
    B, N, _ = points.shape
    with torch.autocast("cuda", enabled=False):
        dist = torch.sqrt(pairwise_distance(points, points))
        k = m.angle_k
        knn = dist.topk(k=k + 1, dim=2, largest=False)[1][:, :, 1:]
        knn_pts = torch.gather(points.unsqueeze(1).expand(B, N, N, 3), 2, knn.unsqueeze(3).expand(B, N, k, 3))
        ref = (knn_pts - points.unsqueeze(2)).unsqueeze(2).expand(B, N, N, k, 3)
        anc = (points.unsqueeze(1) - points.unsqueeze(2)).unsqueeze(3).expand(B, N, N, k, 3)
        sin_v = torch.linalg.norm(torch.cross(ref, anc, dim=-1), dim=-1)
        cos_v = (ref * anc).sum(-1)
        a_idx = torch.atan2(sin_v, cos_v) * m.factor_a
        d_idx = dist / m.sigma_d
        div = m.embedding.div_term

        def sinus(idx):
            om = idx.unsqueeze(-1) * div
            return torch.stack([torch.sin(om), torch.cos(om)], dim=-1).reshape(*idx.shape, -1)

        sd, sa = sinus(d_idx), sinus(a_idx)
    d_emb = _lin(sd, m.proj_d)
    a_emb = _lin(sa, m.proj_a)
    a_emb = a_emb.max(dim=3)[0] if m.reduction_a == "max" else a_emb.mean(dim=3)
    return d_emb + a_emb


def pe_group_mlp_max(pts, radius, nsample, mlp, bf16x3=None, cand_in=None, want_cand=False, out_split=None):
    if bf16x3 is None:
        bf16x3 = torch.is_autocast_enabled() or st.USE_F32X3
    if [tuple(l.conv.weight.shape[:2]) for l in mlp.layers()] != [(32, 6), (64, 32), (128, 64)] or nsample % 32:
        note_fallback("pe_group_mlp_max", f"MLP widths / nsample {nsample} (kernel: 6-32-64-128, nsample % 32 == 0)")
        return pe_group_mlp_max_unfused(pts, radius, nsample, mlp)
    pts = _c(pts.float())
    check_f32(pts, "pts")
    B, N, _ = pts.shape
    cache = getattr(mlp, "_hip_cache", None)
    key = _params_key(mlp)
    if cache is None or cache[0] != key:
        with torch.no_grad():
            flat = []
            for l in mlp.layers():
                w, b = l.folded()
                flat += [w.float().contiguous(), b.float().contiguous()]
        assert [tuple(t.shape) for t in flat[::2]] == [(32, 6), (64, 32), (128, 64)], "kernel is built for [6,32,64,128]"
        from .._lib import lib
        image = torch.empty(lib().unopose_pe_image_bytes(), dtype=torch.uint8, device=pts.device)
        with on_device(pts.device):
            call("unopose_pe_pack_weights", *(ptr(t) for t in flat), ptr(image), stream_ptr())
        cache = (key, flat, image)
        mlp._hip_cache = cache
    w1, b1, w2, b2, w3, b3 = cache[1]
    cand_out = None
    if out_split is not None:
        buf, b0, c0 = out_split
        assert bf16x3 and buf.dtype == torch.bfloat16 and buf.is_contiguous() and buf.shape[1] == N and c0 % 32 == 0 and b0 + B <= buf.shape[0]
        ld = buf.shape[2] // 2
        with on_device(pts.device):
            if want_cand:
                cand_out = (torch.empty(B, N, int(nsample), dtype=torch.int32, device=pts.device),
                            torch.empty(B, N, dtype=torch.int32, device=pts.device))
            ci = cand_in if cand_in is not None else (None, None)
            dst = ctypes.c_void_p(buf.data_ptr() + (b0 * N * ld + c0) * 4)
            call("unopose_pe_group_mlp_max_packed_out", ptr(pts), B, N, float(radius), int(nsample), ptr(cache[2]),
                 None if ci[0] is None else ptr(ci[0]), None if ci[0] is None else ptr(ci[1]),
                 0 if ci[0] is None else int(ci[0].shape[2]), None if cand_out is None else ptr(cand_out[0]),
                 None if cand_out is None else ptr(cand_out[1]), dst, ld, 1, stream_ptr())
        return (buf, cand_out) if want_cand else buf
    out = torch.empty(B, N, 128, dtype=torch.float32, device=pts.device)
    with on_device(pts.device):
        if bf16x3:
            if want_cand:
                cand_out = (torch.empty(B, N, int(nsample), dtype=torch.int32, device=pts.device),
                            torch.empty(B, N, dtype=torch.int32, device=pts.device))
            ci = cand_in if cand_in is not None else (None, None)
            assert ci[0] is None or (ci[0].is_contiguous() and ci[0].shape[:2] == (B, N) and ci[1].shape == (B, N))
            call("unopose_pe_group_mlp_max_packed_cand", ptr(pts), B, N, float(radius), int(nsample), ptr(cache[2]),
                 None if ci[0] is None else ptr(ci[0]), None if ci[0] is None else ptr(ci[1]),
                 0 if ci[0] is None else int(ci[0].shape[2]), None if cand_out is None else ptr(cand_out[0]),
                 None if cand_out is None else ptr(cand_out[1]), ptr(out), stream_ptr())
        else:
            call("unopose_pe_group_mlp_max", ptr(pts), B, N, float(radius), int(nsample), ptr(w1), ptr(b1), ptr(w2),
                 ptr(b2), ptr(w3), ptr(b3), 0, ptr(out), stream_ptr())
    return (out, cand_out) if want_cand else out


def pe_group_mlp_max_unfused(pts, radius, nsample, mlp, chunk=4):
    outs = []
    folded = [l.folded() for l in mlp.layers()]
    with torch.autocast("cuda", enabled=False):
        for b0 in range(0, pts.shape[0], chunk):
            x = query_lrf_group(pts[b0:b0 + chunk], radius, nsample)
            x = x.permute(0, 2, 3, 1)
            for w, b in folded:
                x = F.relu(F.linear(x, w.float(), b.float()))
            outs.append(x.max(dim=2)[0])
    return torch.cat(outs, 0)


def furthest_point_sample(pts, npoint):
    return _ext.furthest_point_sampling(_c(pts.float()), npoint)


def _geo_grid(m, rows, npoint):
    div = m.embedding.div_term
    key = (rows, npoint, div._version, div.data_ptr())
    cache = m.__dict__.setdefault("_geo_grid_cache", {})
    if key not in cache:
        d64 = div.detach().double()
        x = (torch.arange(rows, device=div.device, dtype=torch.float64) - float(npoint // 2 - 1)) / _GEO_HINV
        om = x[:, None] * d64[None, :]
        cache.clear() if len(cache) > 8 else None
        cache[key] = torch.stack([torch.sin(om), torch.cos(om)], dim=-1).reshape(rows, -1)
    return cache[key]


class _GeoEmbedFn(torch.autograd.Function):

    @staticmethod
    def forward(ctx, points, wd, bd, wa, ba, m):
        import math

        npoint = 6
        B, n, _ = points.shape
        rows_a = int(math.floor(math.pi * float(m.factor_a) * _GEO_HINV)) + npoint + 1
        rows_d = _GEO_D_RANGE * _GEO_HINV + npoint
        sd, sa = _geo_grid(m, rows_d, npoint), _geo_grid(m, rows_a, npoint)
        td = (sd @ wd.detach().double().t()).float().contiguous()
        ta = (sa @ wa.detach().double().t()).float().contiguous()
        bias = (bd.detach().float() + ba.detach().float()).contiguous()
        wdf = wd.detach().float().contiguous()
        div = m.embedding.div_term.detach().float().contiguous()
        out = torch.empty(B, n, n, 256, dtype=torch.float32, device=points.device)
        amax = torch.empty(B, n, n, 64, dtype=torch.int32, device=points.device)
        knn = torch.empty(B, n, 3, dtype=torch.int32, device=points.device)
        mean = int(m.reduction_a == "mean")
        with on_device(points.device):
            call("unopose_geo_embedding_train_forward", ptr(points), B, n, ptr(td), rows_d, ptr(ta), rows_a, ptr(bias), ptr(wdf), ptr(div), _GEO_HINV,
                 float(m.sigma_d), float(m.factor_a), mean, ptr(knn), ptr(out), ptr(amax), stream_ptr())
        ctx.save_for_backward(points, knn, amax, sd, sa)
        ctx.meta = (rows_d, rows_a, float(m.sigma_d), float(m.factor_a), mean, npoint)
        return out

    @staticmethod
    def backward(ctx, dE):
        points, knn, amax, sd, sa = ctx.saved_tensors
        rows_d, rows_a, sigma_d, factor_a, mean, npoint = ctx.meta
        B, n, _ = points.shape
        rd_l = min(rows_d, 16 * _GEO_HINV + npoint - 1)
        dE = _c(dE.float())
        G = lib().unopose_geo_embedding_train_workgroups(B, n)
        ws = torch.empty(G, rd_l + rows_a, 256, dtype=torch.float32, device=dE.device)
        full = torch.zeros(rows_d, 256, dtype=torch.float32, device=dE.device)
        past = torch.zeros(1, dtype=torch.int32, device=dE.device)
        with on_device(dE.device):
            call("unopose_geo_embedding_train_backward", ptr(points), ptr(knn), B, n, rows_d, rows_a, _GEO_HINV, sigma_d, factor_a, mean, ptr(dE), ptr(amax),
                 ptr(ws), ptr(full), ptr(past), stream_ptr())
        torch._assert_async(past == 0, "geo embedding backward: a distance index past the table (the clouds are not radius-normalised)")
        dT = ws.double().sum(0)
        dTd = full.double()
        dTd[:rd_l] += dT[:rd_l]
        dTa = dT[rd_l:]
        dwd, dwa = (dTd.t() @ sd).float(), (dTa.t() @ sa).float()
        dbd, dba = dTd.sum(0).float(), dTa.sum(0).float()
        return None, dwd, dbd, dwa, dba, None


def geo_embedding_train_ok(points, m):
    return (st.TRAIN_OWN_GEO and points.is_cuda and m.proj_d.weight.shape == (256, 256) and m.angle_k == 3 and points.shape[1] >= 4
            and m.proj_d.weight.dtype == torch.float32 and not torch.is_autocast_enabled()
            and int(__import__("math").floor(__import__("math").pi * float(m.factor_a) * _GEO_HINV)) + 7 <= 80 - 6)
```

Measured before the change: 1074 pairs/s.

## Split PE grouping into geometry and MLP kernels, sharing ball queries across radii

The fused ball-query, LRF and MLP-max kernel is split in two. A dedicated geometry kernel builds a spatial grid once per cloud, runs both radius ball queries (the second filtered by the first's neighbour list), batches the eigen-decompositions across lanes, and writes u16 neighbour lists and frames. A separate MLP kernel then consumes those precomputed lists and frames. This removes the duplicated grid and ball-query work between the two scales and lets each kernel use its own occupancy, but it adds intermediate global memory traffic and an extra launch.

```diff
diff --git a/include/unopose_hip.h b/include/unopose_hip.h
--- a/include/unopose_hip.h
+++ b/include/unopose_hip.h
@@ -71,16 +71,14 @@
 int unopose_pe_image_bytes(void);
 int unopose_pe_pack_weights(const float *w1, const float *b1, const float *w2, const float *b2,
                             const float *w3, const float *b3, void *image, unopose_stream_t stream);
-int unopose_pe_group_mlp_max_packed(const float *xyz, int B, int N, float radius, int nsample,
-                                    const void *image, float *out, unopose_stream_t stream);
-
-int unopose_pe_group_mlp_max_packed_cand(const float *xyz, int B, int N, float radius, int nsample,
-                                         const void *image, const int *cand_in, const int *cand_cnt_in,
-                                         int cand_stride, int *cand_out, int *cand_cnt_out, float *out,
-                                         unopose_stream_t stream);
-int unopose_pe_group_mlp_max_packed_out(const float *xyz, int B, int N, float radius, int nsample, const void *image,
-                                        const int *cand_in, const int *cand_cnt_in, int cand_stride, int *cand_out,
-                                        int *cand_cnt_out, void *out, int out_ld, int out_split, unopose_stream_t stream);
+
+int unopose_pe_geometry(const float *xyz, int B, int N, float radius, int nsample, float radius2, int nsample2,
+                        const int *cand_in, const int *cand_cnt_in, int cand_stride, void *lists, int *counts,
+                        float *frames, int *cand_out, void *lists2, int *counts2, float *frames2,
+                        unopose_stream_t stream);
+int unopose_pe_mlp_max_packed(const float *xyz, int B, int N, float radius, int nsample, const void *image,
+                              const void *lists, const int *counts, const float *frames, void *out, int out_ld,
+                              int out_split, unopose_stream_t stream);
 
 int unopose_geo_embedding(const float *points, int B, int n, const void *wd_hi,
                           const void *wd_lo, const void *wa_hi, const void *wa_lo,
diff --git a/unopose_amd/_lib.py b/unopose_amd/_lib.py
--- a/unopose_amd/_lib.py
+++ b/unopose_amd/_lib.py
@@ -103,9 +103,8 @@
     "unopose_linear_f32x3": [_P, _P, _P, _P, _P, ctypes.c_long, _I, _I, _I, _P],
     "unopose_pe_image_bytes": [],
     "unopose_pe_pack_weights": [_P, _P, _P, _P, _P, _P, _P, _P],
-    "unopose_pe_group_mlp_max_packed": [_P, _I, _I, _F, _I, _P, _P, _P],
-    "unopose_pe_group_mlp_max_packed_cand": [_P, _I, _I, _F, _I, _P, _P, _P, _I, _P, _P, _P, _P],
-    "unopose_pe_group_mlp_max_packed_out": [_P, _I, _I, _F, _I, _P, _P, _P, _I, _P, _P, _P, _I, _I, _P],
+    "unopose_pe_geometry": [_P, _I, _I, _F, _I, _F, _I, _P, _P, _I, _P, _P, _P, _P, _P, _P, _P, _P],
+    "unopose_pe_mlp_max_packed": [_P, _I, _I, _F, _I, _P, _P, _P, _P, _P, _I, _I, _P],
     "unopose_linear_f32x3_bf16": [_P, _P, _P, _P, _P, ctypes.c_long, _I, _I, _P],
     "unopose_pe_group_mlp_max": [_P, _I, _I, _F, _I, _P, _P, _P, _P, _P, _P, _I, _P, _P],
     "unopose_geo_embedding": [_P, _I, _I, _P, _P, _P, _P, _P, _P, _F, _F, _I, _I, _I, _P, _P, _P],
diff --git a/unopose_amd/csrc/pe.hip b/unopose_amd/csrc/pe.hip
--- a/unopose_amd/csrc/pe.hip
+++ b/unopose_amd/csrc/pe.hip
@@ -1,3 +1,5 @@
+#include <algorithm>
+
 #include "common.h"
 #include "jacobi3.h"
 
@@ -17,24 +19,22 @@
 };
 __device__ __forceinline__ int pe_cell(float v, float o, float ih, int n) { return max(0, min(n - 1, (int)((v - o) * ih))); }
 
-template <typename NT>
-__device__ __forceinline__ int pe_centre_frame(const float *sx, const float *sy, const float *sz, int N, int S,
-                                               float radius, float r2, int lane, float cx, float cy, float cz,
-                                               NT *nbr, Vec3 &xp, Vec3 &yp, Vec3 &zp, const int *cand = nullptr,
-                                               int ncand = -1, const PeGrid *grid = nullptr) {
+template <typename NT, typename CT>
+__device__ __forceinline__ int pe_ball_query(const float *sx, const float *sy, const float *sz, int N, int S, float r2, int lane,
+                                             float cx, float cy, float cz, NT *nbr, const CT *cand, int ncand, const PeGrid &g, bool use_grid) {
   int cnt = 0, first = 0;
-  if (grid && ncand < 0) {
+  if (use_grid && ncand < 0) {
     const int W = (N + 31) >> 5;
-    for (int w = lane; w < W; w += 64) grid->bits[w] = 0u;
-    const int icx = pe_cell(cx, grid->ox, grid->ihx, grid->nx), icy = pe_cell(cy, grid->oy, grid->ihy, grid->ny),
-              icz = pe_cell(cz, grid->oz, grid->ihz, grid->nz);
+    for (int w = lane; w < W; w += 64) g.bits[w] = 0u;
+    const int icx = pe_cell(cx, g.ox, g.ihx, g.nx), icy = pe_cell(cy, g.oy, g.ihy, g.ny),
+              icz = pe_cell(cz, g.oz, g.ihz, g.nz);
     int rs = 0, re = 0;
     if (lane < 9) {
       const int y = icy + lane % 3 - 1, z = icz + lane / 3 - 1;
-      if (y >= 0 && y < grid->ny && z >= 0 && z < grid->nz) {
-        const int row = (z * grid->ny + y) * grid->nx;
-        rs = grid->start[row + max(icx - 1, 0)];
-        re = grid->start[row + min(icx + 1, grid->nx - 1) + 1];
+      if (y >= 0 && y < g.ny && z >= 0 && z < g.nz) {
+        const int row = (z * g.ny + y) * g.nx;
+        rs = g.start[row + max(icx - 1, 0)];
+        re = g.start[row + min(icx + 1, g.nx - 1) + 1];
       }
     }
     __builtin_amdgcn_fence(__ATOMIC_RELEASE, "wavefront");
@@ -44,10 +44,10 @@
     for (int i = 0; i < 9; ++i) {
       const int s0 = __builtin_amdgcn_readlane(rs, i), e0 = __builtin_amdgcn_readlane(re, i);
       for (int q = s0 + lane; q < e0; q += 64) {
-        const int k = grid->order[q];
+        const int k = g.order[q];
         const float x = sx[k], y = sy[k], z = sz[k];
         const float d2 = (cx - x) * (cx - x) + (cy - y) * (cy - y) + (cz - z) * (cz - z);
-        if (d2 < r2) atomicOr(&grid->bits[k >> 5], 1u << (k & 31));
+        if (d2 < r2) atomicOr(&g.bits[k >> 5], 1u << (k & 31));
       }
     }
     __builtin_amdgcn_fence(__ATOMIC_RELEASE, "wavefront");
@@ -55,7 +55,7 @@
     __builtin_amdgcn_fence(__ATOMIC_ACQUIRE, "wavefront");
     for (int w0 = 0; w0 < W; w0 += 64) {
       const int w = w0 + lane;
-      uint32_t bits = w < W ? grid->bits[w] : 0u;
+      uint32_t bits = w < W ? g.bits[w] : 0u;
       const int pc = __builtin_popcount(bits);
       int incl = pc;
 #pragma unroll
@@ -118,8 +118,14 @@
   __builtin_amdgcn_fence(__ATOMIC_RELEASE, "wavefront");
   __builtin_amdgcn_wave_barrier();
   __builtin_amdgcn_fence(__ATOMIC_ACQUIRE, "wavefront");
-
-  float a00 = 0, a01 = 0, a02 = 0, a11 = 0, a12 = 0, a22 = 0;
+  return cnt;
+}
+
+template <typename NT>
+__device__ __forceinline__ void pe_covariance(const float *sx, const float *sy, const float *sz, int S, int lane, float cx, float cy,
+                                              float cz, const NT *nbr, float &a00, float &a01, float &a02, float &a11, float &a12,
+                                              float &a22) {
+  a00 = 0, a01 = 0, a02 = 0, a11 = 0, a12 = 0, a22 = 0;
   for (int l = lane; l < S; l += 64) {
     const int k = nbr[l];
     const float x = cx - sx[k], y = cy - sy[k], z = cz - sz[k];
@@ -128,9 +134,11 @@
   const float inv_s = 1.f / (float)S;
   a00 = wave_sum_f32(a00) * inv_s; a01 = wave_sum_f32(a01) * inv_s; a02 = wave_sum_f32(a02) * inv_s;
   a11 = wave_sum_f32(a11) * inv_s; a12 = wave_sum_f32(a12) * inv_s; a22 = wave_sum_f32(a22) * inv_s;
-  Vec3 e0, e1, z0;
-  float l0, l1, l2;
-  eig_sym3(a00, a01, a02, a11, a12, a22, e0, e1, z0, l0, l1, l2);
+}
+
+template <typename NT>
+__device__ __forceinline__ void pe_frame_axes(const float *sx, const float *sy, const float *sz, int S, float radius, int lane,
+                                              float cx, float cy, float cz, const NT *nbr, Vec3 z0, Vec3 &xp, Vec3 &yp, Vec3 &zp) {
   int vote = 0;
   for (int l0i = 0; l0i < S; l0i += 64) {
     const int l = l0i + lane;
@@ -157,6 +165,19 @@
   const float nacc = sqrtf(vx * vx + vy * vy + vz * vz) + 1e-10f;
   xp = v3(vx / nacc, vy / nacc, vz / nacc);
   yp = cross(xp, zp);
+}
+
+template <typename NT>
+__device__ __forceinline__ int pe_centre_frame(const float *sx, const float *sy, const float *sz, int N, int S,
+                                               float radius, float r2, int lane, float cx, float cy, float cz,
+                                               NT *nbr, Vec3 &xp, Vec3 &yp, Vec3 &zp) {
+  const int cnt = pe_ball_query<NT, int>(sx, sy, sz, N, S, r2, lane, cx, cy, cz, nbr, nullptr, -1, PeGrid{}, false);
+  float a00, a01, a02, a11, a12, a22;
+  pe_covariance(sx, sy, sz, S, lane, cx, cy, cz, nbr, a00, a01, a02, a11, a12, a22);
+  Vec3 e0, e1, z0;
+  float l0, l1, l2;
+  eig_sym3(a00, a01, a02, a11, a12, a22, e0, e1, z0, l0, l1, l2);
+  pe_frame_axes(sx, sy, sz, S, radius, lane, cx, cy, cz, nbr, z0, xp, yp, zp);
   return cnt;
 }
 
@@ -317,24 +338,197 @@
   if (tid < 128) L->b3[tid] = b3[tid];
 }
 
+constexpr int PE_GW = 8;
+constexpr int PE_GB = 4;
+constexpr int PE_GEOM_SCRATCH = PE_GCELLS + 6 * PE_GW + PE_GW;
+
+__device__ __forceinline__ float pe_readlane_f32(float v, int l) { return __int_as_float(__builtin_amdgcn_readlane(__float_as_int(v), l)); }
+
+__global__ __launch_bounds__(PE_GW * 64) void pe_geometry_kernel(
+    const float *__restrict__ xyz, int N, int cpw, float rad0, int S0, float rad1, int S1, const int *__restrict__ cand_in,
+    const int *__restrict__ cand_cnt_in, int cand_stride, u16 *__restrict__ lists0, int *__restrict__ cnt0,
+    float *__restrict__ frames0, int *__restrict__ cand_out, u16 *__restrict__ lists1, int *__restrict__ cnt1,
+    float *__restrict__ frames1, int use_grid) {
+  extern __shared__ float4 smem4[];
+  float *sx = reinterpret_cast<float *>(smem4);
+  float *sy = sx + N, *sz = sy + N;
+  const int BW = use_grid ? (N + 31) >> 5 : 0;
+  uint32_t *bits_all = reinterpret_cast<uint32_t *>(sz + N);
+  u16 *lists_all = reinterpret_cast<u16 *>(bits_all + PE_GW * BW);
+  uint32_t *cnt32 = reinterpret_cast<uint32_t *>(lists_all);
+  float *red = reinterpret_cast<float *>(cnt32 + PE_GCELLS);
+  uint32_t *wtot = reinterpret_cast<uint32_t *>(red + 6 * PE_GW);
+  const int SS = S0 + S1;
+  u16 *gstart = lists_all + max(PE_GW * PE_GB * SS, 2 * PE_GEOM_SCRATCH);
+  u16 *gorder = gstart + PE_GCELLS + 2;
+  const int b = blockIdx.y, tid = threadIdx.x, lane = tid & 63, wave = __builtin_amdgcn_readfirstlane(tid >> 6);
+  const float *P = xyz + (size_t)b * N * 3;
+
+  for (int e = tid; e < N * 3; e += PE_GW * 64) {
+    const float v = P[e];
+    const int p = e / 3, comp = e - p * 3;
+    (comp == 0 ? sx : comp == 1 ? sy : sz)[p] = v;
+  }
+  __syncthreads();
+  PeGrid grid = {};
+  if (use_grid) {
+    float lo[3] = {3e38f, 3e38f, 3e38f}, hi[3] = {-3e38f, -3e38f, -3e38f};
+    for (int p = tid; p < N; p += PE_GW * 64) {
+      lo[0] = fminf(lo[0], sx[p]), hi[0] = fmaxf(hi[0], sx[p]);
+      lo[1] = fminf(lo[1], sy[p]), hi[1] = fmaxf(hi[1], sy[p]);
+      lo[2] = fminf(lo[2], sz[p]), hi[2] = fmaxf(hi[2], sz[p]);
+    }
+#pragma unroll
+    for (int a = 0; a < 3; ++a) {
+      lo[a] = -wave_max_f32(-lo[a]);
+      hi[a] = wave_max_f32(hi[a]);
+      if (lane == 0) red[wave * 6 + a] = lo[a], red[wave * 6 + 3 + a] = hi[a];
+    }
+    for (int c = tid; c < PE_GCELLS; c += PE_GW * 64) cnt32[c] = 0u;
+    __syncthreads();
+    float org[3], ih[3];
+    int nd[3];
+#pragma unroll
+    for (int a = 0; a < 3; ++a) {
+      float l = red[a], h = red[3 + a];
+      for (int w = 1; w < PE_GW; ++w) l = fminf(l, red[w * 6 + a]), h = fmaxf(h, red[w * 6 + 3 + a]);
+      const float ext = h - l, h0 = rad0 * 1.001f;
+      int n = (int)(ext / h0) + 1;
+      float edge = h0;
+      if (!(n <= PE_GDIM)) n = PE_GDIM, edge = fmaxf(h0, ext / (float)PE_GDIM * 1.001f);
+      org[a] = __int_as_float(__builtin_amdgcn_readfirstlane(__float_as_int(l)));
+      ih[a] = __int_as_float(__builtin_amdgcn_readfirstlane(__float_as_int(1.f / edge)));
+      nd[a] = __builtin_amdgcn_readfirstlane(max(n, 1));
+    }
+    grid.ox = org[0], grid.oy = org[1], grid.oz = org[2], grid.ihx = ih[0], grid.ihy = ih[1], grid.ihz = ih[2];
+    grid.nx = nd[0], grid.ny = nd[1], grid.nz = nd[2];
+    grid.start = gstart, grid.order = gorder, grid.bits = bits_all + wave * BW;
+    auto cell_of = [&](int p) {
+      return (pe_cell(sz[p], grid.oz, grid.ihz, grid.nz) * grid.ny + pe_cell(sy[p], grid.oy, grid.ihy, grid.ny)) * grid.nx +
+             pe_cell(sx[p], grid.ox, grid.ihx, grid.nx);
+    };
+    for (int p = tid; p < N; p += PE_GW * 64) atomicAdd(&cnt32[cell_of(p)], 1u);
+    __syncthreads();
+    {
+      static_assert(PE_GW * 64 >= PE_GCELLS && PE_GCELLS % 64 == 0, "one cell per thread");
+      const uint32_t c = tid < PE_GCELLS ? cnt32[tid] : 0u;
+      uint32_t incl = c;
+#pragma unroll
+      for (int d = 1; d < 64; d <<= 1) {
+        const uint32_t t = __shfl_up(incl, d);
+        if (lane >= d) incl += t;
+      }
+      if (lane == 63) wtot[wave] = incl;
+      __syncthreads();
+      if (tid < PE_GCELLS) {
+        uint32_t base = incl - c;
+        for (int w = 0; w < wave; ++w) base += wtot[w];
+        gstart[tid] = (u16)base;
+        cnt32[tid] = base;
+        if (tid == PE_GCELLS - 1) gstart[PE_GCELLS] = (u16)(base + c);
+      }
+    }
+    __syncthreads();
+    for (int p = tid; p < N; p += PE_GW * 64) gorder[atomicAdd(&cnt32[cell_of(p)], 1u)] = (u16)p;
+    __syncthreads();
+  }
+  const float r2_0 = rad0 * rad0, r2_1 = rad1 * rad1;
+  u16 *mylists = lists_all + wave * PE_GB * SS;
+  const int jbase = (blockIdx.x * PE_GW + wave) * cpw;
+
+  for (int c0 = 0; c0 < cpw; c0 += PE_GB) {
+    if (jbase + c0 >= N) break;
+    const int nb = min(PE_GB, min(cpw - c0, N - jbase - c0));
+    float m00 = 0.f, m01 = 0.f, m02 = 0.f, m11 = 0.f, m12 = 0.f, m22 = 0.f;
+#pragma unroll 1
+    for (int i = 0; i < nb; ++i) {
+      const int j = jbase + c0 + i;
+      const size_t row = (size_t)b * N + j;
+      const float cx = sx[j], cy = sy[j], cz = sz[j];
+      u16 *n0 = mylists + i * SS, *n1 = n0 + S0;
+      const int *cand = nullptr;
+      int ncand = -1;
+      if (cand_in) {
+        ncand = cand_cnt_in[row];
+        cand = cand_in + row * cand_stride;
+      }
+      const int c = pe_ball_query<u16, int>(sx, sy, sz, N, S0, r2_0, lane, cx, cy, cz, n0, cand, ncand, grid, use_grid != 0);
+      {
+        uint32_t *dst = reinterpret_cast<uint32_t *>(lists0 + row * S0);
+        const uint32_t *src = reinterpret_cast<const uint32_t *>(n0);
+        for (int l = lane; l < (S0 >> 1); l += 64) dst[l] = src[l];
+        if (cand_out) {
+          int *co = cand_out + row * S0;
+          for (int l = lane; l < S0; l += 64) co[l] = n0[l];
+        }
+        if (lane == 0) cnt0[row] = c <= S0 ? c : -1;
+      }
+      float a00, a01, a02, a11, a12, a22;
+      pe_covariance(sx, sy, sz, S0, lane, cx, cy, cz, n0, a00, a01, a02, a11, a12, a22);
+      if (lane == i) m00 = a00, m01 = a01, m02 = a02, m11 = a11, m12 = a12, m22 = a22;
+      if (S1) {
+        const int c1 = pe_ball_query<u16, u16>(sx, sy, sz, N, S1, r2_1, lane, cx, cy, cz, n1, n0, c <= S0 ? c : -1, grid, use_grid != 0);
+        uint32_t *dst = reinterpret_cast<uint32_t *>(lists1 + row * S1);
+        const uint32_t *src = reinterpret_cast<const uint32_t *>(n1);
+        for (int l = lane; l < (S1 >> 1); l += 64) dst[l] = src[l];
+        if (lane == 0) cnt1[row] = c1 <= S1 ? c1 : -1;
+        pe_covariance(sx, sy, sz, S1, lane, cx, cy, cz, n1, a00, a01, a02, a11, a12, a22);
+        if (lane == PE_GB + i) m00 = a00, m01 = a01, m02 = a02, m11 = a11, m12 = a12, m22 = a22;
+      }
+    }
+    Vec3 e0, e1, z0;
+    float l0, l1, l2;
+    eig_sym3(m00, m01, m02, m11, m12, m22, e0, e1, z0, l0, l1, l2);
+#pragma unroll 1
+    for (int i = 0; i < nb; ++i) {
+      const int j = jbase + c0 + i;
+      const size_t row = (size_t)b * N + j;
+      const float cx = sx[j], cy = sy[j], cz = sz[j];
+      const u16 *n0 = mylists + i * SS, *n1 = n0 + S0;
+#pragma unroll 1
+      for (int sc = 0; sc < (S1 ? 2 : 1); ++sc) {
+        const int src_lane = sc ? PE_GB + i : i;
+        const Vec3 z = v3(pe_readlane_f32(z0.x, src_lane), pe_readlane_f32(z0.y, src_lane), pe_readlane_f32(z0.z, src_lane));
+        Vec3 xp, yp, zp;
+        pe_frame_axes(sx, sy, sz, sc ? S1 : S0, sc ? rad1 : rad0, lane, cx, cy, cz, sc ? n1 : n0, z, xp, yp, zp);
+        const float f = lane == 0 ? xp.x : lane == 1 ? xp.y : lane == 2 ? xp.z : lane == 3 ? yp.x : lane == 4 ? yp.y : lane == 5 ? yp.z
+                        : lane == 6 ? zp.x : lane == 7 ? zp.y : zp.z;
+        if (lane < 9) (sc ? frames1 : frames0)[row * 9 + lane] = f;
+      }
+    }
+    __builtin_amdgcn_wave_barrier();
+  }
+}
+
 constexpr int PE_NW = 4;
 __global__ __launch_bounds__(PE_NW * 64, 8 / PE_NW) void pe_group_mlp_max_bf16x3_kernel(
     const float *__restrict__ xyz, int N, float radius, int S, int cpw, const uint4 *__restrict__ image,
-    const int *__restrict__ cand_in, const int *__restrict__ cand_cnt_in, int cand_stride, int *__restrict__ cand_out,
-    int *__restrict__ cand_cnt_out, float *__restrict__ out, int out_ld, int out_split, int use_grid) {
+    const u16 *__restrict__ lists, const int *__restrict__ counts, const float *__restrict__ frames, float *__restrict__ out,
+    int out_ld, int out_split) {
   extern __shared__ float4 smem4[];
   PeLdsB *L = reinterpret_cast<PeLdsB *>(smem4);
   float *sx = reinterpret_cast<float *>(L + 1);
   float *sy = sx + N, *sz = sy + N;
   float *stage_all = sz + N;
   u16 *nbr_all = reinterpret_cast<u16 *>(stage_all + PE_NW * 128);
-  u16 *gstart = nbr_all + PE_NW * S;
-  u16 *gorder = gstart + PE_GCELLS + 2;
   const int b = blockIdx.y, tid = threadIdx.x, lane = tid & 63, wave = tid >> 6;
   const int half = lane >> 5, col = lane & 31;
   u16 *nbr = nbr_all + wave * S;
   float *stage = stage_all + wave * 128;
   const float *P = xyz + (size_t)b * N * 3;
+  const int SW = S >> 1;
+  const uint32_t *LW = reinterpret_cast<const uint32_t *>(lists) + (size_t)b * N * SW;
+  uint32_t pw0 = 0u, pw1 = 0u;
+  float pf = 0.f;
+  auto fetch = [&](int j) {
+    const uint32_t *p = LW + (size_t)j * SW;
+    pw0 = lane < SW ? p[lane] : 0u;
+    pw1 = lane + 64 < SW ? p[lane + 64] : 0u;
+    const size_t row = (size_t)b * N + j;
+    pf = lane < 9 ? frames[row * 9 + lane] : lane == 9 ? __int_as_float(counts[row]) : 0.f;
+  };
+  const int j0 = (blockIdx.x * PE_NW + wave) * cpw;
+  if (j0 < N) fetch(j0);
 
   for (int e = tid; e < N * 3; e += PE_NW * 64) {
     const float v = P[e];
@@ -343,96 +537,26 @@
   }
   for (int e = tid; e < (int)(sizeof(PeLdsB) / 16); e += PE_NW * 64) smem4[e] = *reinterpret_cast<const float4 *>(image + e);
   __syncthreads();
-  const float r2 = radius * radius;
-  PeGrid grid;
-  if (use_grid) {
-    static_assert(PE_NW * 128 >= PE_GCELLS, "the cell counters borrow the staging area");
-    uint32_t *cnt32 = reinterpret_cast<uint32_t *>(stage_all);
-    float *red = reinterpret_cast<float *>(nbr_all);
-    float lo[3] = {3e38f, 3e38f, 3e38f}, hi[3] = {-3e38f, -3e38f, -3e38f};
-    for (int p = tid; p < N; p += PE_NW * 64) {
-      lo[0] = fminf(lo[0], sx[p]), hi[0] = fmaxf(hi[0], sx[p]);
-      lo[1] = fminf(lo[1], sy[p]), hi[1] = fmaxf(hi[1], sy[p]);
-      lo[2] = fminf(lo[2], sz[p]), hi[2] = fmaxf(hi[2], sz[p]);
-    }
-#pragma unroll
-    for (int a = 0; a < 3; ++a) {
-      lo[a] = -wave_max_f32(-lo[a]);
-      hi[a] = wave_max_f32(hi[a]);
-      if (lane == 0) red[wave * 6 + a] = lo[a], red[wave * 6 + 3 + a] = hi[a];
-    }
-    for (int c = tid; c < PE_GCELLS; c += PE_NW * 64) cnt32[c] = 0u;
-    __syncthreads();
-    float org[3], ih[3];
-    int nd[3];
-#pragma unroll
-    for (int a = 0; a < 3; ++a) {
-      float l = red[a], h = red[3 + a];
-      for (int w = 1; w < PE_NW; ++w) l = fminf(l, red[w * 6 + a]), h = fmaxf(h, red[w * 6 + 3 + a]);
-      const float ext = h - l, h0 = radius * 1.001f;
-      int n = (int)(ext / h0) + 1;
-      float edge = h0;
-      if (!(n <= PE_GDIM)) n = PE_GDIM, edge = fmaxf(h0, ext / (float)PE_GDIM * 1.001f);
-      org[a] = __int_as_float(__builtin_amdgcn_readfirstlane(__float_as_int(l)));
-      ih[a] = __int_as_float(__builtin_amdgcn_readfirstlane(__float_as_int(1.f / edge)));
-      nd[a] = __builtin_amdgcn_readfirstlane(max(n, 1));
-    }
-    grid.ox = org[0], grid.oy = org[1], grid.oz = org[2], grid.ihx = ih[0], grid.ihy = ih[1], grid.ihz = ih[2];
-    grid.nx = nd[0], grid.ny = nd[1], grid.nz = nd[2];
-    grid.start = gstart, grid.order = gorder, grid.bits = reinterpret_cast<uint32_t *>(stage);
-    auto cell_of = [&](int p) {
-      return (pe_cell(sz[p], grid.oz, grid.ihz, grid.nz) * grid.ny + pe_cell(sy[p], grid.oy, grid.ihy, grid.ny)) * grid.nx +
-             pe_cell(sx[p], grid.ox, grid.ihx, grid.nx);
-    };
-    for (int p = tid; p < N; p += PE_NW * 64) atomicAdd(&cnt32[cell_of(p)], 1u);
-    __syncthreads();
-    {
-      constexpr int CPT = PE_GCELLS / (PE_NW * 64);
-      static_assert(CPT * PE_NW * 64 == PE_GCELLS, "cells divide among the threads");
-      uint32_t c[CPT], sum = 0;
-#pragma unroll
-      for (int e = 0; e < CPT; ++e) c[e] = cnt32[tid * CPT + e], sum += c[e];
-      uint32_t incl = sum;
-#pragma unroll
-      for (int d = 1; d < 64; d <<= 1) {
-        const uint32_t t = __shfl_up(incl, d);
-        if (lane >= d) incl += t;
-      }
-      uint32_t *wtot = reinterpret_cast<uint32_t *>(red) + 32;
-      if (lane == 63) wtot[wave] = incl;
-      __syncthreads();
-      uint32_t base = incl - sum;
-      for (int w = 0; w < wave; ++w) base += wtot[w];
-#pragma unroll
-      for (int e = 0; e < CPT; ++e) {
-        gstart[tid * CPT + e] = (u16)base;
-        cnt32[tid * CPT + e] = base;
-        base += c[e];
-      }
-      if (tid == PE_NW * 64 - 1) gstart[PE_GCELLS] = (u16)base;
-    }
-    __syncthreads();
-    for (int p = tid; p < N; p += PE_NW * 64) gorder[atomicAdd(&cnt32[cell_of(p)], 1u)] = (u16)p;
-    __syncthreads();
-  }
 
   for (int ci = 0; ci < cpw; ++ci) {
-    const int j = (blockIdx.x * PE_NW + wave) * cpw + ci;
+    const int j = j0 + ci;
     if (j >= N) break;
     const float cx = sx[j], cy = sy[j], cz = sz[j];
-    Vec3 xp, yp, zp;
-    const int *cand = nullptr;
-    int ncand = -1;
-    if (cand_in) {
-      ncand = cand_cnt_in[(size_t)b * N + j];
-      cand = cand_in + ((size_t)b * N + j) * cand_stride;
-    }
-    const int cnt = pe_centre_frame(sx, sy, sz, N, S, radius, r2, lane, cx, cy, cz, nbr, xp, yp, zp, cand, ncand, use_grid ? &grid : nullptr);
-    if (cand_out) {
-      int *co = cand_out + ((size_t)b * N + j) * S;
-      for (int l = lane; l < S; l += 64) co[l] = nbr[l];
-      if (lane == 0) cand_cnt_out[(size_t)b * N + j] = cnt <= S ? cnt : -1;
-    }
+    {
+      uint32_t *nw = reinterpret_cast<uint32_t *>(nbr);
+      if (lane < SW) nw[lane] = pw0;
+      if (lane + 64 < SW) nw[lane + 64] = pw1;
+      for (int l = lane + 128; l < SW; l += 64) nw[l] = LW[(size_t)j * SW + l];
+    }
+    const Vec3 xp = v3(pe_readlane_f32(pf, 0), pe_readlane_f32(pf, 1), pe_readlane_f32(pf, 2));
+    const Vec3 yp = v3(pe_readlane_f32(pf, 3), pe_readlane_f32(pf, 4), pe_readlane_f32(pf, 5));
+    const Vec3 zp = v3(pe_readlane_f32(pf, 6), pe_readlane_f32(pf, 7), pe_readlane_f32(pf, 8));
+    const int cnt_in = __builtin_amdgcn_readlane(__float_as_int(pf), 9);
+    const int cnt = cnt_in < 0 ? S + 1 : cnt_in;
+    __builtin_amdgcn_fence(__ATOMIC_RELEASE, "wavefront");
+    __builtin_amdgcn_wave_barrier();
+    __builtin_amdgcn_fence(__ATOMIC_ACQUIRE, "wavefront");
+    if (ci + 1 < cpw && j + 1 < N) fetch(j + 1);
 
     f32x16 rmax[4];
 #pragma unroll
@@ -590,44 +714,54 @@
   return check_launch("pe_pack_weights");
 }
 
-int unopose_pe_group_mlp_max_packed(const float *xyz, int B, int N, float radius, int nsample, const void *image,
-                                    float *out, unopose_stream_t stream) {
-  return unopose_pe_group_mlp_max_packed_cand(xyz, B, N, radius, nsample, image, nullptr, nullptr, 0, nullptr, nullptr,
-                                              out, stream);
-}
-
-int unopose_pe_group_mlp_max_packed_cand(const float *xyz, int B, int N, float radius, int nsample, const void *image,
-                                         const int *cand_in, const int *cand_cnt_in, int cand_stride, int *cand_out,
-                                         int *cand_cnt_out, float *out, unopose_stream_t stream) {
-  return unopose_pe_group_mlp_max_packed_out(xyz, B, N, radius, nsample, image, cand_in, cand_cnt_in, cand_stride, cand_out,
-                                             cand_cnt_out, out, 128, 0, stream);
-}
-
-int unopose_pe_group_mlp_max_packed_out(const float *xyz, int B, int N, float radius, int nsample, const void *image,
-                                        const int *cand_in, const int *cand_cnt_in, int cand_stride, int *cand_out,
-                                        int *cand_cnt_out, void *out, int out_ld, int out_split, unopose_stream_t stream) {
-  UNOPOSE_REQUIRE(xyz && image && out, "pe_group_mlp_max_packed: null pointer");
-  UNOPOSE_REQUIRE(out_ld >= 128 && (out_split == 0 || out_split == 1), "pe_group_mlp_max_packed: bad output stride / mode");
-  UNOPOSE_REQUIRE((cand_in == nullptr) == (cand_cnt_in == nullptr) && (cand_out == nullptr) == (cand_cnt_out == nullptr) &&
-                      (!cand_in || cand_stride >= 1),
-                  "pe_group_mlp_max_packed: candidate list and its counts go together");
-  UNOPOSE_REQUIRE(B >= 0 && N >= 1 && nsample >= 32 && nsample % 32 == 0 && B <= 65535,
-                  "pe_group_mlp_max_packed: nsample must be a positive multiple of 32 (got %d)", nsample);
+int unopose_pe_geometry(const float *xyz, int B, int N, float radius, int nsample, float radius2, int nsample2,
+                        const int *cand_in, const int *cand_cnt_in, int cand_stride, void *lists, int *counts, float *frames,
+                        int *cand_out, void *lists2, int *counts2, float *frames2, unopose_stream_t stream) {
+  UNOPOSE_REQUIRE(xyz && lists && counts && frames, "pe_geometry: null pointer");
+  UNOPOSE_REQUIRE((cand_in == nullptr) == (cand_cnt_in == nullptr) && (!cand_in || cand_stride >= 1),
+                  "pe_geometry: candidate list and its counts go together");
+  UNOPOSE_REQUIRE(B >= 0 && N >= 1 && nsample >= 32 && nsample % 32 == 0 && nsample2 >= 0 && nsample2 % 32 == 0 && B <= 65535,
+                  "pe_geometry: nsample must be a positive multiple of 32 (got %d, %d)", nsample, nsample2);
+  UNOPOSE_REQUIRE(nsample2 == 0 || (lists2 && counts2 && frames2 && radius2 <= radius),
+                  "pe_geometry: the second scale needs its outputs and a radius no larger than the first's");
   if (B == 0) return UNOPOSE_OK;
-  size_t lds = sizeof(PeLdsB) + ((size_t)3 * N + PE_NW * 128) * 4 + (size_t)PE_NW * nsample * 2;
-  UNOPOSE_REQUIRE(N < 65536 && lds <= 160 * 1024, "pe_group_mlp_max_packed: N=%d nsample=%d exceed the LDS tile", N, nsample);
-  const size_t grid_bytes = ((size_t)PE_GCELLS + 2 + (size_t)N) * 2;
-  const int use_grid = radius > 0.f && N <= 4096 && N >= 256 && lds + grid_bytes <= 160 * 1024 && (lds + grid_bytes <= 80 * 1024 || lds > 80 * 1024);
+  const size_t lists_bytes = (size_t)2 * std::max(PE_GW * PE_GB * (nsample + nsample2), 2 * PE_GEOM_SCRATCH);
+  size_t lds = (size_t)3 * N * 4 + lists_bytes;
+  const size_t grid_bytes = ((size_t)PE_GCELLS + 2 + (size_t)N) * 2 + (size_t)PE_GW * ((N + 31) >> 5) * 4;
+  UNOPOSE_REQUIRE(N < 65536 && lds <= 160 * 1024, "pe_geometry: N=%d nsample=%d+%d exceed the LDS tile", N, nsample, nsample2);
+  const int use_grid = radius > 0.f && N <= 4096 && N >= 256 && lds + grid_bytes <= 160 * 1024;
   if (use_grid) lds += grid_bytes;
   lds = (lds + 15) & ~(size_t)15;
   static bool opt[64];
-  if (lds_optin(opt, (const void *)pe_group_mlp_max_bf16x3_kernel, 160 * 1024, "pe_group_mlp_max_packed") != UNOPOSE_OK) return UNOPOSE_ELAUNCH;
+  if (lds_optin(opt, (const void *)pe_geometry_kernel, 160 * 1024, "pe_geometry") != UNOPOSE_OK) return UNOPOSE_ELAUNCH;
+  const long centres = (long)B * N;
+  const int cpw = centres >= 16384 ? PE_GB : centres >= 8192 ? 2 : 1;
+  dim3 grid(cdiv(N, PE_GW * cpw), B);
+  hipLaunchKernelGGL(pe_geometry_kernel, grid, dim3(PE_GW * 64), lds, (hipStream_t)stream, xyz, N, cpw, radius, nsample, radius2,
+                     nsample2, cand_in, cand_cnt_in, cand_stride, (u16 *)lists, counts, frames, cand_out, (u16 *)lists2, counts2,
+                     frames2, use_grid);
+  return check_launch("pe_geometry");
+}
+
+int unopose_pe_mlp_max_packed(const float *xyz, int B, int N, float radius, int nsample, const void *image, const void *lists,
+                              const int *counts, const float *frames, void *out, int out_ld, int out_split,
+                              unopose_stream_t stream) {
+  UNOPOSE_REQUIRE(xyz && image && lists && counts && frames && out, "pe_mlp_max_packed: null pointer");
+  UNOPOSE_REQUIRE(out_ld >= 128 && (out_split == 0 || out_split == 1), "pe_mlp_max_packed: bad output stride / mode");
+  UNOPOSE_REQUIRE(B >= 0 && N >= 1 && nsample >= 32 && nsample % 32 == 0 && B <= 65535,
+                  "pe_mlp_max_packed: nsample must be a positive multiple of 32 (got %d)", nsample);
+  if (B == 0) return UNOPOSE_OK;
+  size_t lds = sizeof(PeLdsB) + ((size_t)3 * N + PE_NW * 128) * 4 + (size_t)PE_NW * nsample * 2;
+  UNOPOSE_REQUIRE(N < 65536 && lds <= 160 * 1024, "pe_mlp_max_packed: N=%d nsample=%d exceed the LDS tile", N, nsample);
+  lds = (lds + 15) & ~(size_t)15;
+  static bool opt[64];
+  if (lds_optin(opt, (const void *)pe_group_mlp_max_bf16x3_kernel, 160 * 1024, "pe_mlp_max_packed") != UNOPOSE_OK) return UNOPOSE_ELAUNCH;
   const long centres = (long)B * N;
   const int cpw = centres >= 65536 ? 16 : centres >= 32768 ? 8 : centres >= 8192 ? 4 : centres >= 2048 ? 2 : 1;
   dim3 grid(cdiv(N, PE_NW * cpw), B);
   hipLaunchKernelGGL(pe_group_mlp_max_bf16x3_kernel, grid, dim3(PE_NW * 64), lds, (hipStream_t)stream, xyz, N, radius, nsample,
-                     cpw, (const uint4 *)image, cand_in, cand_cnt_in, cand_stride, cand_out, cand_cnt_out, (float *)out, out_ld, out_split, use_grid);
-  return check_launch("pe_group_mlp_max_packed");
+                     cpw, (const uint4 *)image, (const u16 *)lists, counts, frames, (float *)out, out_ld, out_split);
+  return check_launch("pe_mlp_max_packed");
 }
 
 int unopose_pe_group_mlp_max(const float *xyz, int B, int N, float radius, int nsample, const float *w1,
@@ -645,7 +779,7 @@
   const int cpw = centres >= 32768 ? 8 : centres >= 8192 ? 4 : centres >= 2048 ? 2 : 1;
   dim3 grid(cdiv(N, 4 * cpw), B);
   UNOPOSE_REQUIRE(!bf16x3, "pe_group_mlp_max: the bf16x3 form takes a packed weight image "
-                           "(unopose_pe_pack_weights + unopose_pe_group_mlp_max_packed)");
+                           "(unopose_pe_pack_weights + unopose_pe_geometry + unopose_pe_mlp_max_packed)");
   hipLaunchKernelGGL(pe_group_mlp_max_kernel, grid, dim3(256), lds, (hipStream_t)stream, xyz, N, radius, nsample, cpw,
                      w1, b1, w2, b2, w3, b3, out);
   return check_launch("pe_group_mlp_max");
diff --git a/unopose_amd/model/modules.py b/unopose_amd/model/modules.py
--- a/unopose_amd/model/modules.py
+++ b/unopose_amd/model/modules.py
@@ -530,8 +530,9 @@
                 f2 = self.mlp2.forward_pooled(ops.query_lrf_group(pts, self.r2, self.ns2))
             return torch.cat([f1, f2], dim=1).transpose(1, 2)
         if pts.is_cuda and (torch.is_autocast_enabled() or ops.USE_F32X3) and self.r2 >= self.r1 and self.ns1 % 32 == 0 and self.ns2 % 32 == 0:
-            f2, cand = ops.pe_group_mlp_max(pts, self.r2, self.ns2, self.mlp2, want_cand=True)
-            f1 = ops.pe_group_mlp_max(pts, self.r1, self.ns1, self.mlp1, cand_in=cand)
+            g2, g1, _ = ops.pe_geometry(pts, self.r2, self.ns2, self.r1, self.ns1)
+            f2 = ops.pe_mlp_max(pts, self.r2, self.ns2, self.mlp2, g2)
+            f1 = ops.pe_mlp_max(pts, self.r1, self.ns1, self.mlp1, g1)
         else:
             f1 = ops.pe_group_mlp_max(pts, self.r1, self.ns1, self.mlp1)
             f2 = ops.pe_group_mlp_max(pts, self.r2, self.ns2, self.mlp2)
@@ -543,8 +544,9 @@
 
     def groups_split(self, pts, buf, b0):
         pts = pts.float()
-        _, cand = ops.pe_group_mlp_max(pts, self.r2, self.ns2, self.mlp2, want_cand=True, out_split=(buf, b0, 128))
-        ops.pe_group_mlp_max(pts, self.r1, self.ns1, self.mlp1, cand_in=cand, out_split=(buf, b0, 0))
+        g2, g1, _ = ops.pe_geometry(pts, self.r2, self.ns2, self.r1, self.ns1)
+        ops.pe_mlp_max(pts, self.r2, self.ns2, self.mlp2, g2, out_split=(buf, b0, 128))
+        ops.pe_mlp_max(pts, self.r1, self.ns1, self.mlp1, g1, out_split=(buf, b0, 0))
         return buf
 
     def _mlp3_split(self):
diff --git a/unopose_amd/ops/__init__.py b/unopose_amd/ops/__init__.py
--- a/unopose_amd/ops/__init__.py
+++ b/unopose_amd/ops/__init__.py
@@ -22,7 +22,7 @@
 from .geometry import (
     lrf_global, query_lrf_group, lrf_group_idx, weighted_procrustes, cloud_radius, scale_by_radius, gather_rows, pairwise_distance,
     _bf16_split, _mfma_fragment_order, _GEO_HINV, _GEO_D_RANGE, _GEO_TABLE_UNAVAILABLE, _geo_tables, geo_embedding, geo_embedding_torch,
-    pe_group_mlp_max, pe_group_mlp_max_unfused, furthest_point_sample, _geo_grid, _GeoEmbedFn, geo_embedding_train_ok,
+    pe_group_mlp_max, pe_group_mlp_max_unfused, pe_geometry, pe_mlp_max, _pe_image, furthest_point_sample, _geo_grid, _GeoEmbedFn, geo_embedding_train_ok,
 )
 from .sampling import (
     bilinear_sample_native, sparse_upproj_ok, upproj_plan, sparse_pixel_features, bilinear_sample_pixels,
diff --git a/unopose_amd/ops/geometry.py b/unopose_amd/ops/geometry.py
--- a/unopose_amd/ops/geometry.py
+++ b/unopose_amd/ops/geometry.py
@@ -252,15 +252,30 @@
     return d_emb + a_emb
 
 
-def pe_group_mlp_max(pts, radius, nsample, mlp, bf16x3=None, cand_in=None, want_cand=False, out_split=None):
-    if bf16x3 is None:
-        bf16x3 = torch.is_autocast_enabled() or st.USE_F32X3
-    if [tuple(l.conv.weight.shape[:2]) for l in mlp.layers()] != [(32, 6), (64, 32), (128, 64)] or nsample % 32:
-        note_fallback("pe_group_mlp_max", f"MLP widths / nsample {nsample} (kernel: 6-32-64-128, nsample % 32 == 0)")
-        return pe_group_mlp_max_unfused(pts, radius, nsample, mlp)
+def pe_geometry(pts, radius, nsample, radius2=0.0, nsample2=0, cand_in=None, want_cand=False):
     pts = _c(pts.float())
     check_f32(pts, "pts")
     B, N, _ = pts.shape
+    dev = pts.device
+
+    def bufs(S):
+        return (torch.empty(B, N, int(S), dtype=torch.int16, device=dev), torch.empty(B, N, dtype=torch.int32, device=dev),
+                torch.empty(B, N, 9, dtype=torch.float32, device=dev))
+
+    with on_device(dev):
+        g1 = bufs(nsample)
+        g2 = bufs(nsample2) if nsample2 else None
+        cand = torch.empty(B, N, int(nsample), dtype=torch.int32, device=dev) if want_cand else None
+        ci = cand_in if cand_in is not None else (None, None)
+        assert ci[0] is None or (ci[0].is_contiguous() and ci[0].dtype == torch.int32 and ci[0].shape[:2] == (B, N) and ci[1].shape == (B, N))
+        n2 = (None, None, None) if g2 is None else tuple(ptr(t) for t in g2)
+        call("unopose_pe_geometry", ptr(pts), B, N, float(radius), int(nsample), float(radius2), int(nsample2),
+             None if ci[0] is None else ptr(ci[0]), None if ci[0] is None else ptr(ci[1]), 0 if ci[0] is None else int(ci[0].shape[2]),
+             ptr(g1[0]), ptr(g1[1]), ptr(g1[2]), None if cand is None else ptr(cand), *n2, stream_ptr())
+    return g1, g2, (None if cand is None else (cand, g1[1]))
+
+
+def _pe_image(mlp, dev):
     cache = getattr(mlp, "_hip_cache", None)
     key = _params_key(mlp)
     if cache is None or cache[0] != key:
@@ -271,44 +286,55 @@
                 flat += [w.float().contiguous(), b.float().contiguous()]
         assert [tuple(t.shape) for t in flat[::2]] == [(32, 6), (64, 32), (128, 64)], "kernel is built for [6,32,64,128]"
         from .._lib import lib
-        image = torch.empty(lib().unopose_pe_image_bytes(), dtype=torch.uint8, device=pts.device)
-        with on_device(pts.device):
+        image = torch.empty(lib().unopose_pe_image_bytes(), dtype=torch.uint8, device=dev)
+        with on_device(dev):
             call("unopose_pe_pack_weights", *(ptr(t) for t in flat), ptr(image), stream_ptr())
         cache = (key, flat, image)
         mlp._hip_cache = cache
-    w1, b1, w2, b2, w3, b3 = cache[1]
-    cand_out = None
-    if out_split is not None:
-        buf, b0, c0 = out_split
-        assert bf16x3 and buf.dtype == torch.bfloat16 and buf.is_contiguous() and buf.shape[1] == N and c0 % 32 == 0 and b0 + B <= buf.shape[0]
-        ld = buf.shape[2] // 2
-        with on_device(pts.device):
-            if want_cand:
-                cand_out = (torch.empty(B, N, int(nsample), dtype=torch.int32, device=pts.device),
-                            torch.empty(B, N, dtype=torch.int32, device=pts.device))
-            ci = cand_in if cand_in is not None else (None, None)
+    return cache
+
+
+def pe_mlp_max(pts, radius, nsample, mlp, geom, out_split=None):
+    pts = _c(pts.float())
+    B, N, _ = pts.shape
+    lists, counts, frames = geom
+    assert lists.shape == (B, N, int(nsample)) and counts.shape == (B, N) and frames.shape == (B, N, 9)
+    cache = _pe_image(mlp, pts.device)
+    with on_device(pts.device):
+        if out_split is not None:
+            buf, b0, c0 = out_split
+            assert buf.dtype == torch.bfloat16 and buf.is_contiguous() and buf.shape[1] == N and c0 % 32 == 0 and b0 + B <= buf.shape[0]
+            ld = buf.shape[2] // 2
             dst = ctypes.c_void_p(buf.data_ptr() + (b0 * N * ld + c0) * 4)
-            call("unopose_pe_group_mlp_max_packed_out", ptr(pts), B, N, float(radius), int(nsample), ptr(cache[2]),
-                 None if ci[0] is None else ptr(ci[0]), None if ci[0] is None else ptr(ci[1]),
-                 0 if ci[0] is None else int(ci[0].shape[2]), None if cand_out is None else ptr(cand_out[0]),
-                 None if cand_out is None else ptr(cand_out[1]), dst, ld, 1, stream_ptr())
-        return (buf, cand_out) if want_cand else buf
+            call("unopose_pe_mlp_max_packed", ptr(pts), B, N, float(radius), int(nsample), ptr(cache[2]), ptr(lists), ptr(counts),
+                 ptr(frames), dst, ld, 1, stream_ptr())
+            return buf
+        out = torch.empty(B, N, 128, dtype=torch.float32, device=pts.device)
+        call("unopose_pe_mlp_max_packed", ptr(pts), B, N, float(radius), int(nsample), ptr(cache[2]), ptr(lists), ptr(counts),
+             ptr(frames), ptr(out), 128, 0, stream_ptr())
+    return out
+
+
+def pe_group_mlp_max(pts, radius, nsample, mlp, bf16x3=None, cand_in=None, want_cand=False, out_split=None):
+    if bf16x3 is None:
+        bf16x3 = torch.is_autocast_enabled() or st.USE_F32X3
+    if [tuple(l.conv.weight.shape[:2]) for l in mlp.layers()] != [(32, 6), (64, 32), (128, 64)] or nsample % 32:
+        note_fallback("pe_group_mlp_max", f"MLP widths / nsample {nsample} (kernel: 6-32-64-128, nsample % 32 == 0)")
+        return pe_group_mlp_max_unfused(pts, radius, nsample, mlp)
+    pts = _c(pts.float())
+    check_f32(pts, "pts")
+    B, N, _ = pts.shape
+    if bf16x3:
+        geom, _, cand_out = pe_geometry(pts, radius, nsample, cand_in=cand_in, want_cand=want_cand)
+        out = pe_mlp_max(pts, radius, nsample, mlp, geom, out_split=out_split)
+        return (out, cand_out) if want_cand else out
+    assert out_split is None, "out_split: bf16x3 kernel only"
+    w1, b1, w2, b2, w3, b3 = _pe_image(mlp, pts.device)[1]
     out = torch.empty(B, N, 128, dtype=torch.float32, device=pts.device)
     with on_device(pts.device):
-        if bf16x3:
-            if want_cand:
-                cand_out = (torch.empty(B, N, int(nsample), dtype=torch.int32, device=pts.device),
-                            torch.empty(B, N, dtype=torch.int32, device=pts.device))
-            ci = cand_in if cand_in is not None else (None, None)
-            assert ci[0] is None or (ci[0].is_contiguous() and ci[0].shape[:2] == (B, N) and ci[1].shape == (B, N))
-            call("unopose_pe_group_mlp_max_packed_cand", ptr(pts), B, N, float(radius), int(nsample), ptr(cache[2]),
-                 None if ci[0] is None else ptr(ci[0]), None if ci[0] is None else ptr(ci[1]),
-                 0 if ci[0] is None else int(ci[0].shape[2]), None if cand_out is None else ptr(cand_out[0]),
-                 None if cand_out is None else ptr(cand_out[1]), ptr(out), stream_ptr())
-        else:
-            call("unopose_pe_group_mlp_max", ptr(pts), B, N, float(radius), int(nsample), ptr(w1), ptr(b1), ptr(w2),
-                 ptr(b2), ptr(w3), ptr(b3), 0, ptr(out), stream_ptr())
-    return (out, cand_out) if want_cand else out
+        call("unopose_pe_group_mlp_max", ptr(pts), B, N, float(radius), int(nsample), ptr(w1), ptr(b1), ptr(w2),
+             ptr(b2), ptr(w3), ptr(b3), 0, ptr(out), stream_ptr())
+    return (out, None) if want_cand else out
 
 
 def pe_group_mlp_max_unfused(pts, radius, nsample, mlp, chunk=4):
```

After: 1096 pairs/s, median of 6. +2.1%, better.
